# jimahlstrom/quisk

Measured on AMD Instinct MI355X. Metric: Mcomplex-samples/s through RXA chain, higher is better.
Workload: dtype f64; 1 GPU; 256 channels/GPU x 192 kHz IQ -> 48 kHz SSB RXA chain (shift + 561-tap resample/4 + adc meter + NBP nc 2048 + S meter + fixed AGC + agc meter + panel), 2^22 input samples per channel per step; meters=on, ingest=f64, channels_per_gpu=256, total_channels=256, dsp_size=256, parallelism=channel-sharded x1 (weak), no collective

## Files before the change

include/quiskhip.h:

```cpp
#ifndef QUISKHIP_H
#define QUISKHIP_H

#ifdef __cplusplus
extern "C" {
#endif

typedef enum {
    QH_OK = 0,
    QH_ERR_NO_DEVICE = -1,
    QH_ERR_INVALID = -2,
    QH_ERR_UNSUPPORTED = -3,
    QH_ERR_HIP = -4
} qh_status;

int qh_version(void);
const char *qh_last_error(void);
int qh_device_count(void);

enum { QH_LSB = 0, QH_USB, QH_DSB, QH_CWL, QH_CWU, QH_FM, QH_AM, QH_DIGU, QH_SPEC, QH_DIGL, QH_SAM, QH_DRM };

typedef struct qh_rxa qh_rxa;

qh_rxa *qh_rxa_create(int device, int nch, int dsp_size, int in_rate, int dsp_rate, int out_rate, void *stream);
void qh_rxa_destroy(qh_rxa *e);

int qh_rxa_nch(const qh_rxa *e);
int qh_rxa_dsp_insize(const qh_rxa *e);
int qh_rxa_dsp_outsize(const qh_rxa *e);
void *qh_rxa_stream(const qh_rxa *e);
int qh_rxa_set_graph_replay(qh_rxa *e, int on);
long long qh_rxa_graph_launches(const qh_rxa *e);
int qh_rxa_set_band_tile(qh_rxa *e, int nfft);
int qh_rxa_band_tile(const qh_rxa *e);

int qh_rxa_SetRXAMode(qh_rxa *e, int ch, int mode);
int qh_rxa_RXASetPassband(qh_rxa *e, int ch, double f_low, double f_high);
int qh_rxa_RXASetNC(qh_rxa *e, int ch, int nc);
int qh_rxa_SetRXAShiftRun(qh_rxa *e, int ch, int run);
int qh_rxa_SetRXAShiftFreq(qh_rxa *e, int ch, double fshift);
int qh_rxa_RXANBPSetRun(qh_rxa *e, int ch, int run);
int qh_rxa_RXANBPSetFreqs(qh_rxa *e, int ch, double flow, double fhigh);
int qh_rxa_SetRXABandpassRun(qh_rxa *e, int ch, int run);
int qh_rxa_SetRXABandpassFreqs(qh_rxa *e, int ch, double f_low, double f_high);
int qh_rxa_SetRXAAGCMode(qh_rxa *e, int ch, int mode);
int qh_rxa_SetRXAAGCFixed(qh_rxa *e, int ch, double fixed_agc_db);
int qh_rxa_SetRXAAGCAttack(qh_rxa *e, int ch, int attack_ms);
int qh_rxa_SetRXAAGCDecay(qh_rxa *e, int ch, int decay_ms);
int qh_rxa_SetRXAAGCHang(qh_rxa *e, int ch, int hang_ms);
int qh_rxa_SetRXAAGCTop(qh_rxa *e, int ch, double max_agc_db);
int qh_rxa_SetRXAAGCSlope(qh_rxa *e, int ch, int slope);
int qh_rxa_SetRXAAGCHangThreshold(qh_rxa *e, int ch, int hangthreshold);
int qh_rxa_SetRXAPanelGain1(qh_rxa *e, int ch, double gain);
int qh_rxa_SetRXAPanelGain2(qh_rxa *e, int ch, double gainI, double gainQ);
int qh_rxa_SetRXAPanelSelect(qh_rxa *e, int ch, int select);
int qh_rxa_SetRXAPanelCopy(qh_rxa *e, int ch, int copy);
int qh_rxa_SetRXAAMDSBMode(qh_rxa *e, int ch, int sbmode);
int qh_rxa_SetRXAAMDRun(qh_rxa *e, int ch, int run);
int qh_rxa_SetRXAFMLimRun(qh_rxa *e, int ch, int run);
int qh_rxa_SetRXAFMLimGain(qh_rxa *e, int ch, double gaindB);
int qh_rxa_SetEMNRTables(qh_rxa *e, const double *GG, const double *GGS, const double *zeta_hat, const int *zeta_valid, double gamma_min,
                         double gamma_max, double xi_min, double xi_max);
int qh_rxa_SetRXAEMNRRun(qh_rxa *e, int ch, int run);
int qh_rxa_SetRXAEMNRgainMethod(qh_rxa *e, int ch, int method);
int qh_rxa_SetRXAEMNRnpeMethod(qh_rxa *e, int ch, int method);
int qh_rxa_SetRXAEMNRaeRun(qh_rxa *e, int ch, int run);
int qh_rxa_SetRXAEMNRPosition(qh_rxa *e, int ch, int position);
int qh_rxa_SetRXAEMNRaeZetaThresh(qh_rxa *e, int ch, double v);
int qh_rxa_SetRXAEMNRaePsi(qh_rxa *e, int ch, double v);
int qh_rxa_SetRXAEMNRtrainZetaThresh(qh_rxa *e, int ch, double v);
int qh_rxa_SetRXAEMNRtrainT2(qh_rxa *e, int ch, double v);
int qh_rxa_SetRXAAMSQRun(qh_rxa *e, int ch, int run);
int qh_rxa_SetRXASNBARun(qh_rxa *e, int ch, int run);
int qh_rxa_SetRXASNBAOutputBandwidth(qh_rxa *e, int ch, double flow, double fhigh);
int qh_rxa_SetRXASNBAasize(qh_rxa *e, int ch, int size);
int qh_rxa_SetRXASNBAnpasses(qh_rxa *e, int ch, int npasses);
int qh_rxa_SetRXASNBAk1(qh_rxa *e, int ch, double k1);
int qh_rxa_SetRXASNBAk2(qh_rxa *e, int ch, double k2);
int qh_rxa_SetRXASNBAbridge(qh_rxa *e, int ch, int bridge);
int qh_rxa_SetRXASNBApresamps(qh_rxa *e, int ch, int presamps);
int qh_rxa_SetRXASNBApostsamps(qh_rxa *e, int ch, int postsamps);
int qh_rxa_SetRXASNBApmultmin(qh_rxa *e, int ch, double pmultmin);
int qh_rxa_SetRXASNBAovrlp(qh_rxa *e, int ch, int ovrlp);
int qh_rxa_SetRXACBLRun(qh_rxa *e, int ch, int run);
int qh_rxa_SetRXASPCWRun(qh_rxa *e, int ch, int run);
int qh_rxa_SetRXASPCWFreq(qh_rxa *e, int ch, double freq);
int qh_rxa_SetRXASPCWBandwidth(qh_rxa *e, int ch, double bw);
int qh_rxa_SetRXASPCWGain(qh_rxa *e, int ch, double gain);
int qh_rxa_SetRXAmpeakRun(qh_rxa *e, int ch, int run);
int qh_rxa_SetRXAmpeakNpeaks(qh_rxa *e, int ch, int npeaks);
int qh_rxa_SetRXAmpeakFilEnable(qh_rxa *e, int ch, int fil, int enable);
int qh_rxa_SetRXAmpeakFilFreq(qh_rxa *e, int ch, int fil, double freq);
int qh_rxa_SetRXAmpeakFilBw(qh_rxa *e, int ch, int fil, double bw);
int qh_rxa_SetRXAmpeakFilGain(qh_rxa *e, int ch, int fil, double gain);
int qh_rxa_SetRXASSQLRun(qh_rxa *e, int ch, int run);
int qh_rxa_SetRXASSQLThreshold(qh_rxa *e, int ch, double threshold);
int qh_rxa_SetRXASSQLTauMute(qh_rxa *e, int ch, double tau_mute);
int qh_rxa_SetRXASSQLTauUnMute(qh_rxa *e, int ch, double tau_unmute);
int qh_rxa_SetRXAFMSQRun(qh_rxa *e, int ch, int run);
int qh_rxa_SetRXAFMSQThreshold(qh_rxa *e, int ch, double threshold);
int qh_rxa_SetRXAFMSQNC(qh_rxa *e, int ch, int nc);
int qh_rxa_SetRXAFMSQMP(qh_rxa *e, int ch, int mp);
int qh_rxa_SetRXAEQRun(qh_rxa *e, int ch, int run);
int qh_rxa_SetRXAEQNC(qh_rxa *e, int ch, int nc);
int qh_rxa_SetRXAEQMP(qh_rxa *e, int ch, int mp);
int qh_rxa_SetRXAEQProfile(qh_rxa *e, int ch, int nfreqs, const double *F, const double *G);
int qh_rxa_SetRXAEQCtfmode(qh_rxa *e, int ch, int mode);
int qh_rxa_SetRXAEQWintype(qh_rxa *e, int ch, int wintype);
int qh_rxa_SetRXAGrphEQ(qh_rxa *e, int ch, const int *rxeq);
int qh_rxa_SetRXAGrphEQ10(qh_rxa *e, int ch, const int *rxeq);
int qh_rxa_SetRXAAMSQThreshold(qh_rxa *e, int ch, double threshold_db);
int qh_rxa_SetRXAAMSQMaxTail(qh_rxa *e, int ch, double tail_seconds);
int qh_rxa_SetRXAANFRun(qh_rxa *e, int ch, int v);
int qh_rxa_SetRXAANFTaps(qh_rxa *e, int ch, int v);
int qh_rxa_SetRXAANFDelay(qh_rxa *e, int ch, int v);
int qh_rxa_SetRXAANFPosition(qh_rxa *e, int ch, int v);
int qh_rxa_SetRXAANFGain(qh_rxa *e, int ch, double v);
// ... 681 lines not shown
```

quisk_amd/csrc/qh_engine.hip:

```cpp
#include "qh_engine.hpp"

namespace qh {

void launch_egress_pack(const double2 *src, long long src_stride, int nch, long long n, const EgressFmt &f, hipStream_t s)
{
    const long long per = (n + 255) / 256;
    hipLaunchKernelGGL(egress_pack_kernel, dim3((unsigned)(per < 1024 ? per : 1024), (unsigned)nch), dim3(256), 0, s, src, src_stride,
                       (int)n, f);
}

void Engine::pack_audio(const double2 *src, long long src_stride, long long n)
{
    launch_egress_pack(src, src_stride, nch, n, eg, stream);
}

void Engine::tick(int cat)
{
    if (!timing) return;
    if (ev_used >= (int)ev.size()) {
        hipEvent_t e;
        (void)hipEventCreate(&e);
        ev.push_back(e);
        ev_cat.push_back(0);
    }
    ev_cat[(size_t)ev_used] = cat;
    (void)hipEventRecord(ev[(size_t)ev_used], stream);
    ev_used++;
}

template <int D, bool MIX, bool PACKED = false, bool METER = false, bool OUTMIX = false, bool EGRESS = false, int NFFT = kNfft, bool POLY = false,
          int DET = 0, bool PAIR = false, bool MROW = false>
static void launch_osfir(OsfirArgs<double> a, int ntiles, int nch, hipStream_t s)
{
    a.ntiles = ntiles;
    dim3 grid((unsigned)ntiles * (unsigned)nch), block(NT);
    constexpr int lds = osfir_lds_bytes<double, NFFT, D, METER>();
    hipLaunchKernelGGL((osfir_kernel<double, NFFT, D, MIX, PACKED, METER, OUTMIX, EGRESS, POLY, DET, PAIR, MROW>), grid, block, lds, s, a);
}
template <int NFFT>
static void launch_band_rows(OsfirArgs<double> a, int ntiles, int nch, hipStream_t s)
{
    launch_osfir<1, false, false, false, false, false, NFFT, false, 0, false, true>(a, ntiles, nch, s);
}
template <int NFFT>
static void launch_band(OsfirArgs<double> a, int ntiles, int nch, hipStream_t s, bool meter, bool egress)
{
    if (meter && egress) launch_osfir<1, false, false, true, false, true, NFFT>(a, ntiles, nch, s);
    else if (meter) launch_osfir<1, false, false, true, false, false, NFFT>(a, ntiles, nch, s);
    else if (egress) launch_osfir<1, false, false, false, false, true, NFFT>(a, ntiles, nch, s);
    else launch_osfir<1, false, false, false, false, false, NFFT>(a, ntiles, nch, s);
}

static void launch_band6k(OsfirArgs<double> a, int ntiles, int nch, hipStream_t s, bool meter, bool egress)
{
    a.ntiles = ntiles;
    dim3 grid((unsigned)ntiles * (unsigned)nch), block(kOsfir6kThreads);
    constexpr int lds = osfir6k_lds_bytes();
    if (a.mask_row) hipLaunchKernelGGL((osfir6k_kernel<false, false, true>), grid, block, lds, s, a);
    else if (meter && egress) hipLaunchKernelGGL((osfir6k_kernel<true, true>), grid, block, lds, s, a);
    else if (meter) hipLaunchKernelGGL((osfir6k_kernel<true, false>), grid, block, lds, s, a);
    else if (egress) hipLaunchKernelGGL((osfir6k_kernel<false, true>), grid, block, lds, s, a);
    else hipLaunchKernelGGL((osfir6k_kernel<false, false>), grid, block, lds, s, a);
}

static void launch_band2g(OsfirArgs<double> a, int ntiles, int nch, hipStream_t s, bool meter, bool egress)
{
    a.ntiles = ntiles;
    dim3 grid((unsigned)ntiles * (unsigned)nch), block(kOsfir8kThreads);
    constexpr int lds = osfir8k_lds_bytes();
    if (a.mask_row) hipLaunchKernelGGL((osfir8k_kernel<false, false, true>), grid, block, lds, s, a);
    else if (meter && egress) hipLaunchKernelGGL((osfir8k_kernel<true, true>), grid, block, lds, s, a);
    else if (meter) hipLaunchKernelGGL((osfir8k_kernel<true, false>), grid, block, lds, s, a);
    else if (egress) hipLaunchKernelGGL((osfir8k_kernel<false, true>), grid, block, lds, s, a);
    else hipLaunchKernelGGL((osfir8k_kernel<false, false>), grid, block, lds, s, a);
}

int Engine::tile_lds_limits()
{
#define QH_SET_LDS(D, ...) QH_HIP(hipFuncSetAttribute(reinterpret_cast<const void *>(&osfir_kernel<double, 4096, D, __VA_ARGS__>), \
                                                     hipFuncAttributeMaxDynamicSharedMemorySize, (osfir_lds_bytes<double, 4096, D, true>())))
    QH_SET_LDS(1, false); QH_SET_LDS(1, false, false, true);
    QH_SET_LDS(1, false, false, false, false, true); QH_SET_LDS(1, false, false, true, false, true);
    QH_SET_LDS(1, false, false, false, false, false, false, 0, false, true); QH_SET_LDS(1, false, false, false, false, false, false, 0, true, true);
#define QH_SET_LDS8(...) QH_HIP(hipFuncSetAttribute(reinterpret_cast<const void *>(&osfir_kernel<double, kBandNfftMax, 1, false, false, __VA_ARGS__>), \
                                                     hipFuncAttributeMaxDynamicSharedMemorySize, (osfir_lds_bytes<double, kBandNfftMax, 1, true>())))
    QH_SET_LDS8(false, false, false); QH_SET_LDS8(true, false, false); QH_SET_LDS8(false, false, true); QH_SET_LDS8(true, false, true);
    QH_SET_LDS8(false, false, false, false, 0, false, true);
#undef QH_SET_LDS8
#define QH_SET_LDS6K(...) QH_HIP(hipFuncSetAttribute(reinterpret_cast<const void *>(&osfir6k_kernel<__VA_ARGS__>), \
        hipFuncAttributeMaxDynamicSharedMemorySize, osfir6k_lds_bytes()))
    QH_SET_LDS6K(false, false); QH_SET_LDS6K(true, false); QH_SET_LDS6K(false, true); QH_SET_LDS6K(true, true); QH_SET_LDS6K(false, false, true);
#undef QH_SET_LDS6K
#define QH_SET_LDS2G(...) QH_HIP(hipFuncSetAttribute(reinterpret_cast<const void *>(&osfir8k_kernel<__VA_ARGS__>), \
                                                      hipFuncAttributeMaxDynamicSharedMemorySize, osfir8k_lds_bytes()))
    QH_SET_LDS2G(false, false); QH_SET_LDS2G(true, false); QH_SET_LDS2G(false, true); QH_SET_LDS2G(true, true); QH_SET_LDS2G(false, false, true);
#undef QH_SET_LDS2G
    QH_SET_LDS(2, false, false, false, true, false, true); QH_SET_LDS(4, false, false, false, true, false, true); QH_SET_LDS(8, false, false, false, true, false, true);
    QH_SET_LDS(2, false, true, false, true, false, true); QH_SET_LDS(4, false, true, false, true, false, true); QH_SET_LDS(8, false, true, false, true, false, true);
#undef QH_SET_LDS
    if (D > 1) QH_HIP(hipFuncSetAttribute(reinterpret_cast<const void *>(&front_mask_kernel<kNfft>), hipFuncAttributeMaxDynamicSharedMemorySize,
                                          (TileFft<kNfft, false, double2>::kLdsBytes)));
    return QH_OK;
}

int Engine::emnr_lds_limit()
{
    QH_HIP(hipFuncSetAttribute(reinterpret_cast<const void *>(&emnr_kernel), hipFuncAttributeMaxDynamicSharedMemorySize, emnr_lds_bytes()));
    return QH_OK;
}

void Engine::launch_nco_retune(int n)
{
    hipLaunchKernelGGL(nco_retune_hist_kernel, dim3((kHistFront + NT - 1) / NT, (unsigned)n), dim3(NT), 0, stream,
                       hist_front[cur_front], kHistFront, nco_phase, nco_dphase, nco_parked, (const int *)retune_list,
                       (const unsigned long long *)retune_law);
}

void Engine::launch_nco_park(int ch, int run)
{
    hipLaunchKernelGGL(nco_park_kernel, dim3(1), dim3(1), 0, stream, nco_phase, nco_parked, ch, run);
}

void Engine::launch_front_masks(int n)
{
    hipLaunchKernelGGL((front_mask_kernel<kNfft>), dim3((unsigned)n), dim3(NT), (size_t)(TileFft<kNfft, false, double2>::kLdsBytes),
                       stream, (const double *)front_taps, front_ntaps, (const unsigned long long *)nco_dphase, (const int *)retune_list, front_fold,
                       (const double2 *)tw4096, mask_front, lane_rot, nco_step, 1);
}

void Engine::launch_ssql_flush()
{
    hipLaunchKernelGGL(ssql_flush_kernel, dim3((unsigned)nch), dim3(64), 0, stream, ssql_state);
}

void Engine::launch_fmsq_flush()
{
    hipLaunchKernelGGL(fmsq_flush_kernel, dim3((unsigned)((nch + 63) / 64)), dim3(64), 0, stream, fq_state, nch, fq_nready);
}

int Engine::run_front(const double2 *src, long long src_stride, double2 *dst, long long dst_stride, const EpiParam *ep,
                      long long n_in, long long n_mid, const int *list, int nlist, int part)
{
    if (part == 0) tick(0);
    if (D > 1) {
        OsfirArgs<double> a{};
        a.in = src; a.in_stride = src_stride;
        a.hist = hist_front[cur_front]; a.hist_stride = kHistFront; a.hist_len = kHistFront;
        a.out = dst; a.out_stride = dst_stride; a.out_offset = 0;
        a.mask = mask_front; a.mask_stride = kNfft;
        a.tw_fwd = tw4096; a.tw_inv = tw_inv_front;
        a.nco_step = nco_step; a.lane_rot = lane_rot;
        a.epi = ep;
        a.n_in = (int)n_in; a.n_out = (int)n_mid; a.off = 0; a.P = front_P; a.Lout = front_L; a.pick = front_pick;
        const int per_tile = front_L / front_pick;
        const int ntiles = (int)((n_mid + per_tile - 1) / per_tile);
        a.chan_list = list;
        const int nl = list ? nlist : nch;
        if (part <= 1) if (int rc = grow(tile_rot, tile_rot_cap, ntiles, nch)) return rc;
        if (part <= 1) hipLaunchKernelGGL(nco_tile_kernel, dim3((unsigned)((ntiles + 255) / 256), (unsigned)nch), dim3(256), 0, stream,
                           (const unsigned long long *)nco_phase, (const unsigned long long *)nco_dphase, tile_rot, ntiles,
                           (long long)(a.off - a.P), (long long)front_fold * front_L);
        a.tile_rot = tile_rot;
        a.pk_src = pk_src; a.pk = pk;
        const bool hist_in_kernel = !pk_src && n_in >= kHistFront && n_mid > 0;
        if (hist_in_kernel) a.hist_next = hist_front[cur_front ^ 1];
        if (part == 1 || part == 3) { }
        else if (pk_src) {
            switch (front_fold) {
            case 2: launch_osfir<2, false, true, false, true, false, kNfft, true>(a, ntiles, nl, stream); break;
            case 4: launch_osfir<4, false, true, false, true, false, kNfft, true>(a, ntiles, nl, stream); break;
            case 8: launch_osfir<8, false, true, false, true, false, kNfft, true>(a, ntiles, nl, stream); break;
            default: return set_error(QH_ERR_UNSUPPORTED, "decimation %d not supported", D);
            }
        } else {
            switch (front_fold) {
            case 2: launch_osfir<2, false, false, false, true, false, kNfft, true>(a, ntiles, nl, stream); break;
            case 4: launch_osfir<4, false, false, false, true, false, kNfft, true>(a, ntiles, nl, stream); break;
            case 8: launch_osfir<8, false, false, false, true, false, kNfft, true>(a, ntiles, nl, stream); break;
            default: return set_error(QH_ERR_UNSUPPORTED, "decimation %d not supported", D);
            }
        }
        if (part == 0) tick(2);
        if (part == 1 || part == 2) return QH_OK;
        dim3 g((kHistFront + NT - 1) / NT, (unsigned)nch);
        if (pk_src)
            hipLaunchKernelGGL((hist_update_kernel<double, false, true>), g, dim3(NT), 0, stream, src, src_stride, (int)n_in,
                               hist_front[cur_front], hist_front[cur_front ^ 1], kHistFront, (const unsigned long long *)nullptr,
                               (const unsigned long long *)nullptr, (const int *)nullptr, pk_src, pk);
        else if (!hist_in_kernel)
            hipLaunchKernelGGL((hist_update_kernel<double, false>), g, dim3(NT), 0, stream, src, src_stride, (int)n_in,
                               hist_front[cur_front], hist_front[cur_front ^ 1], kHistFront, (const unsigned long long *)nullptr,
                               (const unsigned long long *)nullptr, (const int *)nullptr, (const unsigned char *)nullptr, PackedFmt{});
        cur_front ^= 1;
    } else if (D == 0) {
        if (pk_src) return set_error(QH_ERR_UNSUPPORTED, "packed input needs in_rate / dsp_rate in 2, 4, 8, 16");
        if (int rc = grow(fbuf, fbuf_cap, n_in, nch)) return rc;
        long long per = (n_in + NT - 1) / NT;
        dim3 g((unsigned)(per < 4096 ? per : 4096), (unsigned)nch);
        hipLaunchKernelGGL((pointwise_kernel<double, true>), g, dim3(NT), 0, stream, src, src_stride, fbuf, fbuf_cap,
                           (int)n_in, nco_phase, nco_dphase, (const EpiParam *)nullptr, (const int *)nullptr);
        int got = 0;
        if (int rc = qh_rat_process(rsmpin, fbuf, fbuf_cap, (int)n_in, dst, dst_stride, &got)) return rc;
        if (got != (int)n_mid) return set_error(QH_ERR_HIP, "input resampler produced %d samples, expected %lld", got, n_mid);
        if (ep) {
            long long pm = (n_mid + NT - 1) / NT;
            hipLaunchKernelGGL((pointwise_kernel<double, false>), dim3((unsigned)(pm < 1024 ? pm : 1024), (unsigned)nch), dim3(NT), 0, stream,
                               (const double2 *)dst, dst_stride, dst, dst_stride, (int)n_mid, (const unsigned long long *)nullptr,
                               (const unsigned long long *)nullptr, ep, (const int *)nullptr);
        }
        tick(2);
    } else {
        if (pk_src) return set_error(QH_ERR_UNSUPPORTED, "packed input needs in_rate > dsp_rate (unpack with qh_unpack_iq first)");
        long long per = (n_in + NT - 1) / NT;
        dim3 g((unsigned)(per < 4096 ? per : 4096), (unsigned)nch);
        hipLaunchKernelGGL((pointwise_kernel<double, true>), g, dim3(NT), 0, stream, src, src_stride, dst, dst_stride,
                           (int)n_in, nco_phase, nco_dphase, ep, (const int *)nullptr);
        tick(2);
    }
    hipLaunchKernelGGL(nco_advance_kernel, dim3((nch + 255) / 256), dim3(256), 0, stream, nco_phase, nco_dphase, nch, n_in);
    return QH_OK;
}

static __global__ __launch_bounds__(NT) void long_gather_kernel(const double2 *hist, const double2 *src, long long src_stride, int n, double2 *cat,
                                                                long long cat_stride, const int *chan_list, int lh)
{
    const int ch = chan_list ? chan_list[blockIdx.y] : (int)blockIdx.y;
    const double2 *h = hist + (long long)ch * kLongHist, *x = src + (long long)ch * src_stride;
    double2 *c = cat + (long long)ch * cat_stride;
    const long long tot = (long long)kLongHist + n;
    for (long long i = (long long)(kLongHist - lh) + (long long)blockIdx.x * NT + threadIdx.x; i < tot; i += (long long)gridDim.x * NT) c[i] = i < kLongHist ? h[i] : x[i - kLongHist];
}
static __global__ __launch_bounds__(NT) void long_hist_kernel(const double2 *cat, long long cat_stride, int n, double2 *hist, const int *chan_list, int lh)
{
    const int ch = chan_list ? chan_list[blockIdx.y] : (int)blockIdx.y;
    const double2 *c = cat + (long long)ch * cat_stride + n;
    double2 *h = hist + (long long)ch * kLongHist;
    for (int i = kLongHist - lh + blockIdx.x * NT + threadIdx.x; i < kLongHist; i += gridDim.x * NT) h[i] = c[i];
}
static __global__ __launch_bounds__(NT) void long_add_kernel(double2 *dst, long long dst_stride, const double2 *add, long long add_stride, int n, const int *chan_list,
                                                             const int *row_parts, int row_stride, const int *mask_row, int p)
{
    const int ch = chan_list ? chan_list[blockIdx.y] : (int)blockIdx.y;
    if (p >= row_parts[mask_row ? (long long)mask_row[ch] : (long long)ch * row_stride]) return;
    double2 *d = dst + (long long)ch * dst_stride;
    const double2 *a = add + (long long)ch * add_stride;
    for (int i = blockIdx.x * NT + threadIdx.x; i < n; i += gridDim.x * NT) { d[i].x += a[i].x; d[i].y += a[i].y; }
}

static __global__ __launch_bounds__(NT) void long_migrate_kernel(double2 *hist, double2 *lhist, int to_long)
{
    const int ch = blockIdx.y;
    double2 *h = hist + (long long)ch * kHistBand, *l = lhist + (long long)ch * kLongHist;
    for (int i = blockIdx.x * NT + threadIdx.x; i < kLongHist; i += gridDim.x * NT) {
        const int j = i - (kLongHist - kHistBand);
        if (to_long) l[i] = j >= 0 ? h[j] : make_double2(0.0, 0.0);
        else if (j >= 0) h[j] = l[i];
    }
}

void Engine::run_band(const double2 *src, long long src_stride, double2 *dst, long long dst_stride, const EpiParam *ep,
// ... 7 lines not shown
        const int K = f.parts, Pk = kLongPart - 1, Lk = kBandNfftMax - Pk, nt = (int)((n_mid + Lk - 1) / Lk);
        const int nl = list ? nlist : nch;
        const long long cat_stride = kLongHist + lcat_cap;
        const int lh = K * kLongPart - 1;
        const long long per = (lh + n_mid + NT - 1) / NT;
        tick(1);
        hipLaunchKernelGGL(long_gather_kernel, dim3((unsigned)(per < 2048 ? per : 2048), (unsigned)nl), dim3(NT), 0, stream, (const double2 *)f.lhist[hc], src,
                           src_stride, (int)n_mid, lcat, cat_stride, list, lh);
        for (int p = 0; p < K; p++) {
            OsfirArgs<double> a{};
            a.in = lcat + kLongHist - (long long)kLongPart * p; a.in_stride = cat_stride;
            a.hist = a.in - Pk; a.hist_stride = cat_stride; a.hist_len = Pk;
            a.out = p ? ltmp : dst; a.out_stride = p ? lcat_cap : dst_stride; a.out_offset = 0;
            a.mask = f.lmask + (size_t)p * kBandNfftMax; a.mask_stride = f.mask_stride ? (long long)kLongParts * kBandNfftMax : 0;
            a.mask_row = f.mask_row;
            a.tw_fwd = a.tw_inv = tw8192;
            a.tw_r2 = tw8192 + 32;
            a.chan_list = list;
            a.n_in = (int)n_mid; a.n_out = (int)n_mid; a.off = 0; a.P = Pk; a.Lout = Lk;
            if (f.mask_row) launch_band_rows<kBandNfftMax>(a, nt, nl, stream);
            else launch_band<kBandNfftMax>(a, nt, nl, stream, false, false);
            const long long pn = (n_mid + NT - 1) / NT;
            if (p) hipLaunchKernelGGL(long_add_kernel, dim3((unsigned)(pn < 1024 ? pn : 1024), (unsigned)nl), dim3(NT), 0, stream, dst, dst_stride,
                                      (const double2 *)ltmp, lcat_cap, (int)n_mid, list, (const int *)f.lrow_parts, f.mask_stride ? 1 : 0, (const int *)f.mask_row, p);
        }
        const long long pn = (n_mid + NT - 1) / NT;
        if (ep) hipLaunchKernelGGL((pointwise_kernel<double, false>), dim3((unsigned)(pn < 1024 ? pn : 1024), (unsigned)nl), dim3(NT), 0, stream,
                                   (const double2 *)dst, dst_stride, dst, dst_stride, (int)n_mid, (const unsigned long long *)nullptr,
                                   (const unsigned long long *)nullptr, ep, list);
        tick(2);
        hipLaunchKernelGGL(long_hist_kernel, dim3(64, (unsigned)nl), dim3(NT), 0, stream, (const double2 *)lcat, cat_stride, (int)n_mid, f.lhist[hc ^ 1], list, lh);
        return;
    }
    const int Lout = bnfft - P;
    const int ntiles = (int)((n_mid + Lout - 1) / Lout);
    OsfirArgs<double> a{};
    a.in = src; a.in_stride = src_stride;
    a.hist = hist[hc]; a.hist_stride = kHistBand; a.hist_len = kHistBand;
    a.out = dst; a.out_stride = dst_stride; a.out_offset = 0;
    a.mask = f.mask; a.mask_stride = f.mask_stride;
    a.mask_row = f.mask_row;
    a.tw_fwd = a.tw_inv = (bnfft == kNfft || band2g) ? tw4096 : tw8192;
    a.tw_r2 = tw8192 + 32;
    a.epi = ep;
    a.chan_list = list;
    a.n_in = (int)n_mid; a.n_out = (int)n_mid; a.off = 0; a.P = P; a.Lout = Lout;
    tick(1);
    if (meter) { a.meter_in = m_part[0]; a.meter_out = m_part[1]; a.meter_stride = m_part_cap; a.meter_w = m_w; }
    if (egress) a.eg = eg;
    const int nl = list ? nlist : nch;
    const bool hist_in_kernel = !pairs && (det || (!band6k && !band2g)) && n_mid >= kHistBand;
    if (hist_in_kernel) a.hist_next = hist[hc ^ 1];
    if (pairs) {
        a.chan_list = pairs;
        if (band_fmdc) {
            a.fmdc_a = band_fmdc->a; a.fmdc_stride = band_fmdc->stride; a.fmdc_shift = band_fmdc->shift;
            a.fmdc_cin = fm_cin; a.fmdc_cstride = fm_cin_cap; a.fmdc_pw = fm_pw; a.fmdc_gain = fm_again;
        }
        if (band_amlv) {
            a.amlv_a = band_amlv->a; a.amlv_stride = band_amlv->stride; a.amlv_shift = band_amlv->shift;
            a.amlv_cin = am_cin; a.amlv_cstride = am_cin_cap; a.amlv_pw = am_pw;
        }
        if (a.mask_row) launch_osfir<1, false, false, false, false, false, kNfft, false, 0, true, true>(a, ntiles, npairs, stream);
        else launch_osfir<1, false, false, false, false, false, kNfft, false, 0, true>(a, ntiles, npairs, stream);
    } else if (det) {
        a.det_out = det_out; a.det_stride = det_stride;
        if (det == 2 || det == 3) {
            a.det_sum = am_tsum; a.det_sum_stride = am_tsum_cap;
            a.det_m[0] = am_prm.mtauR; a.det_m[1] = am_prm.mtauI;
            a.det_m256[0] = std::pow(am_prm.mtauR, 256.0); a.det_m256[1] = std::pow(am_prm.mtauI, 256.0);
            a.det_g[0] = am_prm.onem_mtauR; a.det_g[1] = am_prm.onem_mtauI;
            a.det_lf = levelfade; a.det_last = am_last; a.det_scan = am_pw + 2 * 2048;
            for (int f = 0; f < 2; f++) {
                const double m = a.det_m[f];
                a.det_mp[f][0] = m; a.det_mp[f][1] = m * m; a.det_mp[f][2] = (m * m) * (m * m); a.det_mp[f][3] = ((m * m) * (m * m)) * ((m * m) * (m * m));
            }
            if (det == 3) launch_osfir<1, false, false, false, false, false, kNfft, false, 3>(a, ntiles, nl, stream);
            else launch_osfir<1, false, false, false, false, false, kNfft, false, 2>(a, ntiles, nl, stream);
        } else launch_osfir<1, false, false, false, false, false, kNfft, false, 1>(a, ntiles, nl, stream);
    } else if (band6k) launch_band6k(a, ntiles, nl, stream, meter, egress);
    else if (band2g) launch_band2g(a, ntiles, nl, stream, meter, egress);
    else if (a.mask_row && bnfft == kNfft) launch_band_rows<kNfft>(a, ntiles, nl, stream);
    else if (a.mask_row) launch_band_rows<kBandNfftMax>(a, ntiles, nl, stream);
    else if (bnfft == kNfft) launch_band<kNfft>(a, ntiles, nl, stream, meter, egress);
    else launch_band<kBandNfftMax>(a, ntiles, nl, stream, meter, egress);
    tick(2);
    dim3 g((kHistBand + NT - 1) / NT, (unsigned)(list ? nlist : nch));
    if (pairs && band_amlv)
        hipLaunchKernelGGL(am_audio_hist_kernel, g, dim3(256), 0, stream, band_amlv->a, band_amlv->stride, (int)n_mid, list, (const double *)am_cin, am_cin_cap,
                           (const double *)am_pw, band_amlv->shift, (const double2 *)hist[hc], hist[hc ^ 1], kHistBand);
    else if (pairs && band_fmdc)
        hipLaunchKernelGGL(fm_audio_hist_kernel, g, dim3(256), 0, stream, band_fmdc->a, band_fmdc->stride, (int)n_mid, list, (const double *)fm_cin, fm_cin_cap,
                           (const double *)fm_pw, band_fmdc->shift, (const double *)fm_again, (const double2 *)hist[hc], hist[hc ^ 1], kHistBand);
    else if (!hist_in_kernel)
        hipLaunchKernelGGL((hist_update_kernel<double, false>), g, dim3(NT), 0, stream, src, src_stride, (int)n_mid,
                           hist[hc], hist[hc ^ 1], kHistBand, (const unsigned long long *)nullptr,
                           (const unsigned long long *)nullptr, list);
}

int Engine::process(const double *d_in, long long in_stride, double *d_out, long long out_stride, int nblk)
{
    if (!rsmpout) return process_chain(d_in, in_stride, d_out, out_stride, nblk);
    if (nblk <= 0) return QH_OK;
    QH_HIP(hipSetDevice(device));
    if (eg.kind) {
        const long long n_out = (long long)nblk * dsp_outsize;
        if (int rc = ensure_abuf(n_out)) return rc;
        const EgressFmt keep = eg;
        eg = EgressFmt{};
        const int rc = process(d_in, in_stride, reinterpret_cast<double *>(abuf), abuf_cap, nblk);
        eg = keep;
        if (rc) return rc;
        pack_audio(abuf, abuf_cap, n_out);
        QH_HIP(hipGetLastError());
        return QH_OK;
    }
    const long long n_mid = (long long)nblk * dsp_size;
    if (int rc = grow(obuf, obuf_cap, n_mid, nch)) return rc;
    if (int rc = process_chain(d_in, in_stride, reinterpret_cast<double *>(obuf), obuf_cap, nblk)) return rc;
    int got = 0;
    if (int rc = qh_rat_process(rsmpout, obuf, obuf_cap, (int)n_mid, d_out, out_stride, &got)) return rc;
    if (got != nblk * dsp_outsize) return set_error(QH_ERR_HIP, "output resampler produced %d samples, expected %d", got, nblk * dsp_outsize);
    return QH_OK;
}

static bool extents_apart(const double2 *a, long long a_stride, long long a_n, const double2 *b, long long b_stride, long long b_n, int nch)
{
    const double2 *a_end = a + (size_t)(nch - 1) * (size_t)a_stride + (size_t)a_n, *b_end = b + (size_t)(nch - 1) * (size_t)b_stride + (size_t)b_n;
    return (const char *)a_end <= (const char *)b || (const char *)b_end <= (const char *)a;
}

int Engine::chain_needs(ChainCall &k)
{
    for (const ChanCfg &c : cfg) {
        if (c.agc_run && c.agc_mode > 4)
            return set_error(QH_ERR_UNSUPPORTED, "AGC mode %d is not provided (0 fixed, 1-4 long/slow/med/fast)", c.agc_mode);
        if (c.amd_run && c.fmd_run) return set_error(QH_ERR_UNSUPPORTED, "channel %d: the AM and the FM detector both switched on", (int)(&c - cfg.data()));
        if (c.amd_run || c.fmd_run || (c.agc_run && c.agc_mode != 0) || c.lms[0].run || c.lms[1].run || c.amsq_run || c.emnr_run || c.snba_run || c.ap_on() || c.ssql_on()) k.mixed = true;
        if (c.sender_run || c.sip_run) k.mixed = k.taps = true;
        if (c.gen_run) {
            if (c.gen_mode == 4 || c.gen_mode == 5)
                return set_error(QH_ERR_UNSUPPORTED, "channel %d: gen0 mode %d (%s) is not provided", (int)(&c - cfg.data()), c.gen_mode, c.gen_mode == 4 ? "sawtooth" : "triangle");
            k.mixed = k.gen = true;
        }
        if (c.ssql_on() && ((int)(0.070 * dsp_rate) < 64))
            return set_error(QH_ERR_UNSUPPORTED, "SSQL needs ramps of 64 samples or more: dsp_rate %d is too low", dsp_rate);
        if (c.emnr_run && !emnr_tables) return set_error(QH_ERR_INVALID, "EMNR needs its gain tables first (qh_rxa_SetEMNRTables: WDSP's `calculus` and `zetaHat.bin` data)");
        if (c.nbp_run) { k.any_nbp = true; if (c.nbp_nc > k.nc_max) k.nc_max = c.nbp_nc; } else k.every_nbp = false;
        if (c.bp1_run) { k.any_bp1 = true; if (c.bp1_nc > k.nc_max) k.nc_max = c.bp1_nc; }
        if (c.fmd_run) {
            k.nc_max = std::max({ k.nc_max, c.fm_nc_de, c.fm_nc_aud });
            if (1.1 * c.fm_f_high >= 0.5 * (double)dsp_rate)
                return set_error(QH_ERR_UNSUPPORTED, "channel %d: FM audio band up to %g Hz needs 1.1 * high below dsp_rate / 2 = %g", (int)(&c - cfg.data()),
                                 c.fm_f_high, 0.5 * (double)dsp_rate);
        }
        if (c.fmsq_run) {
            const int ch = (int)(&c - cfg.data());
            if (!c.fmd_run) return set_error(QH_ERR_UNSUPPORTED, "channel %d: FMSQ runs while the FM detector is off", ch);
            if ((double)dsp_rate <= 2.0 * fm_pllpole(1.0, 20000.0))
                return set_error(QH_ERR_UNSUPPORTED, "FMSQ needs a dsp rate above twice the FM loop's pole frequency (%.0f Hz): %d is too low",
                                 2.0 * fm_pllpole(1.0, 20000.0), dsp_rate);
            if (c.fmsq_nc > kLongPart) return set_error(QH_ERR_UNSUPPORTED, "channel %d: FMSQ nc = %d exceeds %d", ch, c.fmsq_nc, kLongPart);
            if (c.fmsq_nc > k.nc_max) k.nc_max = c.fmsq_nc;
        }
    }
    for (const ChanCfg &c : cfg) {
        if (!c.eqp_run) continue;
// ... 47 lines not shown
        if (f.dirty) for (ChanCfg &c : cfg) c.*f.dirty = true;
        else fm_dirty = fm_relayout = true;
    }
    return QH_OK;
}

void Engine::pick_band_tile(int nc_max)
{
    const bool two_group = nc_max <= 2048 && band_tile_pref == 8192;
    const bool six_k = nc_max <= 2048 && band_tile_pref == 6144;
    const int want = six_k ? kOsfir6kN : (nc_max > 2048 || two_group) ? kBandNfftMax : kNfft;
    if (want != bnfft || two_group != band2g || six_k != band6k) {
        bnfft = want; band2g = two_group; band6k = six_k;
        for (ChanCfg &c : cfg) { c.nbp_dirty = c.bp1_dirty = true; c.snb_dirty = true; }
    }
}

int Engine::process_chain(const double *d_in, long long in_stride, double *d_out, long long out_stride, int nblk)
{
    if (nblk <= 0) return QH_OK;
    QH_HIP(hipSetDevice(device));
    ChainCall k;
    k.nblk = nblk;
    if (int rc = chain_needs(k)) return rc;
    if (int rc = plan_long(k)) return rc;
    pick_band_tile(k.nc_max);
    k.meters_fused = meters_on && !k.mixed && k.any_nbp && !k.any_bp1 && !k.any_eqp && dsp_size >= 64 && dsp_size <= 2048 && !k.long_mode;
    if (meters_on && !k.meters_fused) k.mixed = true;
    if (meters_on) if (int rc = meters_alloc()) return rc;
    if (int rc = refresh_params()) return rc;
    if (k.mixed) if (int rc = refresh_demod()) return rc;
    if (k.gen) if (int rc = refresh_gen()) return rc;
    if (!k.mixed && k.any_bp1) {
        std::vector<int> run;
        for (int ch = 0; ch < nch; ch++) if (cfg[(size_t)ch].bp1_run) run.push_back(ch);
        if (int rc = fc_follow(fc[FC_BP1], run)) return rc;
    }
    if (lists[L_SNBA].n) if (int rc = refresh_params()) return rc;
    if (k.any_eqp || eq_lists_dirty) if (int rc = refresh_eqp()) return rc;

    k.n_in = (long long)nblk * dsp_insize;
    k.n_mid = (long long)nblk * dsp_size;
    if (k.n_in > 0x7fffffffLL) return set_error(QH_ERR_INVALID, "too many samples in one call");
    if (int rc = ensure_buffers(k.n_mid)) return rc;
    if (k.long_mode) if (int rc = long_buffers()) return rc;
    if (int rc = refresh_ap(k)) return rc;
    if (int rc = refresh_ssql(k)) return rc;
    if (fq_list.n) if (int rc = grow(fq_noise, fq_noise_cap, buf_cap, nch)) return rc;
    if (k.taps && tap_lists[0].n) if (int rc = grow(snd_rows, snd_cap, buf_cap, nch)) return rc;
    snd_n = k.taps && tap_lists[0].n ? k.n_mid : 0;
    ev_used = 0;

    k.in = reinterpret_cast<const double2 *>(d_in); k.in_stride = in_stride;
    k.out = reinterpret_cast<double2 *>(d_out); k.out_stride = out_stride;
    k.P = band6k ? kOsfir6kP : band2g ? kOsfir8kP : k.meters_fused ? ((k.nc_max - 1 + 255) / 256) * 256 : k.long_mode ? kLongPart - 1 : k.nc_max - 1;
    k.eg_fused = eg.kind && (k.mixed ? lists[L_AMSQ].n == 0 : ((k.any_nbp || k.any_bp1 || k.any_eqp) && !k.long_mode));
    if (eg.kind && !k.eg_fused) {
        if (int rc = ensure_abuf(k.n_mid)) return rc;
        k.out = abuf; k.out_stride = abuf_cap;
    }
    if (!k.mixed) return run_linear(k);

    if (int rc = plan_mixed(k)) return rc;
    if (int rc = run_mixed_front(k)) return rc;
    if (int rc = run_am(k)) return rc;
    if (k.side) QH_HIP(hipEventRecord(ev_join, side_stream));
    if (lists[L_FM].n) if (int rc = run_fm(k)) return rc;
    if (k.side) QH_HIP(hipStreamWaitEvent(stream, ev_join, 0));
    if (lists[L_SNB + 1].n) snb_inplace(k, lists[L_SNB + 1].dev, lists[L_SNB + 1].n);
    if (lists[L_SNB].n || lists[L_SNB + 1].n) fc[FC_SNB].flip();
    if (int rc = run_snba(k)) return rc;
    eqp_inplace(k);
    lms_at(k, 0, k.cur);
    bp1_at(k, 0);
    tick(1);
    if (lists[L_AGC_CUR].n || lists[L_AGC_OTHER].n) if (int rc = run_agc(k)) return rc;
    run_output(k);
    QH_HIP(hipGetLastError());
    return QH_OK;
}

int Engine::run_linear(ChainCall &k)
{
    const long long n_mid = k.n_mid;
    const int nstage = 1 + (k.any_nbp ? 1 : 0) + (k.any_eqp ? 1 : 0) + (k.any_bp1 ? 1 : 0);
    int stage = 0, which = 0;
    const double2 *cur = k.in;
    long long cur_stride = k.in_stride;
    auto dst_of = [&](int st, long long &stride) -> double2 * {
        if (st == nstage - 1) { stride = k.out_stride; return k.out; }
        stride = buf_cap;
        double2 *p = buf[which];
        which ^= 1;
        return p;
    };
    {
        long long dst_stride;
        double2 *dst = dst_of(stage, dst_stride);
        const bool over = nstage == 1 && !extents_apart(k.out, k.out_stride, n_mid, k.in, k.in_stride, k.n_in, nch);
        if (over) { dst = buf[0]; dst_stride = buf_cap; }
        if (int rc = run_front(cur, cur_stride, dst, dst_stride, stage == nstage - 1 ? epi : nullptr, k.n_in, n_mid)) return rc;
        if (over) QH_HIP(hipMemcpy2DAsync(k.out, (size_t)k.out_stride * sizeof(double2), dst, (size_t)dst_stride * sizeof(double2),
                                          (size_t)n_mid * sizeof(double2), (size_t)nch, hipMemcpyDeviceToDevice, stream));
        cur = dst; cur_stride = dst_stride; stage++;
    }
    for (int f = 0; f < 3; f++) {
        if (f == 0 ? !k.any_nbp : f == 1 ? !k.any_eqp : !k.any_bp1) continue;
        long long dst_stride;
        double2 *dst = dst_of(stage, dst_stride);
        if (f == 1) {
            const bool last = stage == nstage - 1;
            run_band(cur, cur_stride, dst, dst_stride, last ? epi : nullptr, n_mid, fc[FC_EQP], k.P, eq_list.dev, eq_list.n, false, k.eg_fused && last);
            fc[FC_EQP].flip();
            if (eq_rest.n) {
                const long long per = (n_mid + NT - 1) / NT;
                const dim3 g((unsigned)(per < 1024 ? per : 1024), (unsigned)eq_rest.n);
                if (!last) hipLaunchKernelGGL(copy_rows_kernel, g, dim3(NT), 0, stream, cur, dst, buf_cap, (int)n_mid, (const int *)eq_rest.dev);
                else {
                    auto *pass = k.eg_fused ? &pointwise_kernel<double, false, true> : &pointwise_kernel<double, false>;
                    hipLaunchKernelGGL(pass, g, dim3(NT), 0, stream, cur, cur_stride, dst, dst_stride, (int)n_mid, (const unsigned long long *)nullptr,
                                       (const unsigned long long *)nullptr, (const EpiParam *)epi, (const int *)eq_rest.dev, k.eg_fused ? eg : EgressFmt{});
                }
            }
            cur = dst; cur_stride = dst_stride; stage++;
            continue;
        }
        if (k.meters_fused) if (int rc = ensure_meter_partials(n_mid, bnfft - k.P)) return rc;
        Fircore &band = fc[f == 0 ? FC_NBP : FC_BP1];
        run_band(cur, cur_stride, dst, dst_stride, stage == nstage - 1 ? epi : nullptr, n_mid, band, k.P, nullptr, 0, k.meters_fused, k.eg_fused && stage == nstage - 1);
        band.flip();
        cur = dst; cur_stride = dst_stride; stage++;
    }
    if (k.meters_fused)
        hipLaunchKernelGGL(meter_finish_kernel, dim3((unsigned)nch), dim3(kMeterFinishThreads), 0, stream, m_part[0], m_part[1],
                           m_part_cap, (int)(n_mid / 64), dsp_size / 64, (bnfft - k.P) / 64, band6k ? 2 : band2g ? 1 : 0, m_adc, m_s, m_agc,
                           -1.0 / ((double)dsp_rate * 0.100), -1.0 / ((double)dsp_rate * 0.100), (const double *)m_g2);
    if (eg.kind && !k.eg_fused) pack_audio(k.out, k.out_stride, n_mid);
    tick(3);
    QH_HIP(hipGetLastError());
    return QH_OK;
}

int Engine::plan_mixed(ChainCall &k)
{
    k.split = lists[L_FM].n > 0 && lists[L_REST].n > 0 && D > 1 && !meters_on && !k.taps && !k.gen && !lists[L_AMSQ].n && !lists[L_SNB].n && !timing && !(dbg_forms & 1);
    k.fm_theta_fused = k.split && k.any_nbp && !band6k && !band2g && bnfft == kNfft && !(dbg_forms & 8);
    bool no_lms = true;
    for (int f = 0; f < 2; f++) for (int p = 0; p < 3; p++) no_lms = no_lms && !lms_n(3 * f + p);
    k.direct = k.split && !(dbg_forms & 2) && !eq_list.n && k.every_nbp && !eg.kind && !lists[L_LIM].n && !lists[L_AGC_CUR].n && !lists[L_AGC_OTHER].n && !lists[L_SNBA].n && !lists[L_SNB + 1].n && no_lms &&
               !lists[L_EMNR].n && !lists[L_EMNR + 1].n && !lists[L_EMNR + 2].n && !lists[L_FIX].n && !lists[L_FIX + 1].n && !lists[L_BP1P + 1].n && lists[L_BP1P].n == lists[L_BP1].n && lists[L_RB].n == lists[L_BP1].n &&
               lists[L_USB].n + lists[L_FM].n == lists[L_PLAIN].n && !lists[L_AP].n && !lists[L_AP + 1].n && !ssql_listed() &&
               extents_apart(k.out, k.out_stride, k.n_mid, k.in, k.in_stride, k.n_in, nch);
    k.P_am = ((k.P + 63) / 64) * 64;
    k.am_fused = k.direct && !(dbg_forms & 4) && lists[L_AM].n > 0 && lists[L_RB].n == lists[L_AM].n + lists[L_SAM].n && !band6k && !band2g && bnfft == kNfft && k.P_am < bnfft;
    k.am_lv_fused = k.am_fused && k.P_am == 2048 && bnfft - k.P_am == 2048 && np_am > 0 && lists[L_BP1P].n && fc[FC_BP1].parts <= 1 && !(dbg_forms & (16 | 512));
    k.side = k.split || ((lists[L_AM].n || lists[L_SAM].n) && lists[L_FM].n && !(dbg_forms & 32));
    if (k.am_fused) {
        if (int rc = grow(am_tsum, am_tsum_cap, (k.n_mid + (bnfft - k.P_am) - 1) / (bnfft - k.P_am), 2LL * nch)) return rc;
        if (k.am_lv_fused) if (int rc = grow(am_cin, am_cin_cap, am_tsum_cap + 1, 2LL * nch)) return rc;
    }
    if (k.side) if (int rc = ensure_side_stream()) return rc;
    for (double *&q : seg_sum)
        if (!q) if (int rc = alloc(q, (long long)nch * kSegWaves * kSegMaxGroups * kSegSumW)) return rc;
    k.cur = buf[0]; k.other = buf[1];
    return QH_OK;
}
// ... 664 lines not shown
```

quisk_amd/csrc/qh_engine.hpp:

```cpp
#pragma once
#include <hip/hip_runtime.h>
#include <algorithm>
#include <cmath>
#include <cstdarg>
#include <cstdio>
#include <cstdlib>
#include <cstring>
#include <map>
#include <mutex>
#include <string>
#include <vector>
#include "../../include/quiskhip.h"
#include "qh_design.hpp"
#pragma clang diagnostic push
#pragma clang diagnostic ignored "-Wunused-function"
#include "qh_kernels.hpp"
#include "qh_demod.hpp"
#include "qh_tiled.hpp"
#include "qh_agc_tiled.hpp"
#include "qh_emnr.hpp"
#include "qh_snba.hpp"
#include "qh_audio_peak.hpp"
#include "qh_ssql.hpp"
#include "qh_fmsq.hpp"
// ... 65 lines not shown
    int bp1_pos = 0;
    bool demod_dirty = true, ctcss_flush = false;
    bool nbp_dirty = true, bp1_dirty = true, nco_dirty = true, epi_dirty = true;
    bool nbp_flush = false, bp1_flush = false;
    int cbl_run = 0, sp_run = 0, mp_run = 0, mp_npeaks = 2;
    double sp_f = 600.0, sp_bw = 100.0, sp_gain = 2.0;
    int mp_enable[kApPeaks] = { 1, 1 };
    double mp_f[kApPeaks] = { 2125.0, 2295.0 }, mp_bw[kApPeaks] = { 75.0, 75.0 }, mp_gain[kApPeaks] = { 1.0, 1.0 };
    bool ap_dirty = true, sp_flush = false, mp_flush[kApPeaks] = { false, false };
    bool ap_on() const { return cbl_run || sp_run || mp_run; }
    int ssql_run = 0;
    double ssql_wthresh = 0.08, ssql_tau_mute = 0.1, ssql_tau_unmute = 0.1;
    bool ssql_dirty = true;
    bool ssql_on() const { return ssql_run != 0; }
    int fmsq_run = 0, fmsq_nc = 2048, fmsq_mp = 0;
    double fmsq_tail_thresh = 0.750, fmsq_unmute_thresh = 0.562;
    bool fmsq_dirty = true;
    int eqp_run = 0, eqp_nc = 2048, eqp_mp = 0, eqp_ctfmode = 0, eqp_wintype = 0;
    std::vector<double> eqp_F = { 0.0, 32.0, 63.0, 125.0, 250.0, 500.0, 1000.0, 2000.0, 4000.0, 8000.0, 16000.0 }, eqp_G = std::vector<double>(11, 0.0);
    bool eqp_dirty = true, eqp_flush = false, eqp_tie = false;
    int sender_run = 0, sip_run = 0;
    int gen_run = 0, gen_mode = 2;
    double gen_tone_mag = 1.0, gen_tone_freq = 1000.0, gen_noise_mag = 1.0;
    double gen_sweep_mag = 1.0, gen_sweep_f1 = -20000.0, gen_sweep_f2 = 20000.0, gen_sweep_rate = 4000.0;
    unsigned long long gen_seed = 0;
    bool gen_seed_set = false, gen_dirty = true, gen_sweep_dirty = true, gen_tone_reset = false, gen_sweep_reset = false;
    bool fix_before() const
    {
        return agc_run && agc_mode == 0 && ((bp1_run && bp1_pos) || (lms[0].run && lms[0].position) || (lms[1].run && lms[1].position) ||
                                            (emnr_run && emnr_pos) || ap_on() || ssql_on());
    }
};

enum FcId { FC_NBP, FC_BP1, FC_DE, FC_AUD, FC_SNB, FC_FQ, FC_EQP, FC_COUNT };

struct Fircore {
    double2 *mask = nullptr;
    long long mask_stride = 0;
    bool by_design = false;
    int rows = 1;
    int *mask_row = nullptr;
    long long mask_rows(int nch) const { return by_design ? rows : mask_stride ? nch : 1; }
    double2 *hist[2] = { nullptr, nullptr };
    int cur = 0;
    bool ChanCfg::*dirty = nullptr;
    bool can_long = true;
    int parts = 1;
    double2 *lmask = nullptr, *lhist[2] = { nullptr, nullptr };
    int *lrow_parts = nullptr;
    struct Chan { bool listed = false, long_live = false; int at = 0; };
    std::vector<Chan> chan;
    bool carried = false;
    void flip() { cur ^= 1; }
};

struct Engine {
    int device = 0, nch = 0, dsp_size = 0, in_rate = 0, dsp_rate = 0, out_rate = 0;
    int D = 1, dsp_insize = 0, dsp_outsize = 0, front_fold = 1, front_pick = 1;
    unsigned long long epoch = 0;
    struct GraphKey {
        const void *in = nullptr; void *out = nullptr; long long in_stride = 0, out_stride = 0; int nblk = 0;
        unsigned long long epoch = ~0ull;
        bool operator==(const GraphKey &o) const
        { return in == o.in && out == o.out && in_stride == o.in_stride && out_stride == o.out_stride && nblk == o.nblk && epoch == o.epoch; }
    };
    struct GraphSlot { hipGraphExec_t exec = nullptr; unsigned after = 0; };
    bool graph_on = false, graph_seen = false;
    GraphKey graph_key;
    GraphSlot graph_slot[256];
    long long graph_launches = 0;
    hipStream_t stream = nullptr;
    bool own_stream = false;
    hipStream_t side_stream = nullptr;
    hipEvent_t ev_fork = nullptr, ev_join = nullptr;
    std::vector<ChanCfg> cfg;
    int front_ntaps = 0, front_P = 0, front_L = 0;
    double2 *mask_front = nullptr;
    double2 *tw4096 = nullptr, *tw_inv_front = nullptr, *tw8192 = nullptr;
    int bnfft = kNfft;
    bool band2g = false;
    bool band6k = false;
    int dbg_forms = [] { const char *e = std::getenv("QH_DBG_FORMS"); return e ? std::atoi(e) : 0; }();
    int band_tile_pref = 0;
    std::vector<cd> band_mask(const std::vector<cd> &h) const;
    unsigned long long *nco_phase = nullptr, *nco_dphase = nullptr, *nco_parked = nullptr;
    double2 *nco_step = nullptr;
    double2 *lane_rot = nullptr, *tile_rot = nullptr;
    long long tile_rot_cap = 0;
    double *front_taps = nullptr;
    int *retune_list = nullptr;
    unsigned long long *retune_law = nullptr;
    EpiParam *epi = nullptr;
    double2 *hist_front[2] = { nullptr, nullptr };
    int cur_front = 0;
    Fircore fc[FC_COUNT];
    double2 *buf[2] = { nullptr, nullptr };
    long long buf_cap = 0;
    double2 *lcat = nullptr, *ltmp = nullptr;
    long long lcat_cap = 0;
    int long_stage_alloc(Fircore &f);
    int long_buffers();
    int long_masks_upload(Fircore &f, long long row, const std::vector<cd> &h);
    std::map<void *, long long> owned;
    long long dev_bytes() const { long long b = 0; for (const auto &o : owned) b += o.second; return b; }
    bool timing = false;
    std::vector<hipEvent_t> ev;
    std::vector<int> ev_cat;
    int ev_used = 0;
    double last_ms[3] = { 0, 0, 0 };

    bool demod_alloc = false, lists_dirty = true;
    enum ListId {
        L_AM, L_SAM, L_FM, L_BP1, L_PLAIN, L_AGC_CUR, L_AGC_OTHER, L_LMS, L_BP1P = L_LMS + 6, L_FIX = L_BP1P + 2, L_AMSQ = L_FIX + 2, L_EMNR,
        L_SNB = L_EMNR + 3, L_SNBA = L_SNB + 2,
        L_REST,
        L_USB, L_RB,
        L_LIM, L_AP, L_PAIRS_FM = L_AP + 2, L_PAIRS_AM, L_PAIRS_SAM, L_COUNT
    };
    struct ChanList { int *dev = nullptr; int n = 0; };
    ChanList lists[L_COUNT];
    int *list_block = nullptr;
    int np_fm = 0, np_am = 0, np_sam = 0;
    bool de_real = false;
    bool all_nbp = false;
    int n_sam0 = 0;
    double *fix_gain = nullptr;
    ApParam *ap_prm = nullptr;
    double *ap_state = nullptr, *ap_M = nullptr, *ap_ends = nullptr;
    long long ap_ends_cap = 0;
    int ap_L = 0;
    std::vector<double> ap_M_h;
    std::vector<ApParam> ap_prm_h;
    int ap_alloc();
    ChanList ssql_lists[2];
    std::vector<int> ssql_h[2];
    int *ssql_list_block = nullptr;
    SsqlParam *ssql_prm = nullptr;
    SsqlState *ssql_state = nullptr;
    double *ssql_cup = nullptr, *ssql_cdown = nullptr, *ssql_ends = nullptr;
    unsigned long long *ssql_bits = nullptr;
    int *ssql_rec = nullptr;
    long long ssql_ends_cap = 0, ssql_wcap = 0, ssql_rec_cap = 0;
    int ssql_L = 0, ssql_ntup = 0, ssql_ntdown = 0;
    std::vector<SsqlParam> ssql_prm_h;
    int ssql_alloc();
    bool ssql_listed() const { return ssql_lists[0].n || ssql_lists[1].n; }
    ChanList fq_list, fq_pairs;
    std::vector<int> fq_h, fq_pairs_h;
    int *fq_list_block = nullptr;
    int np_fq = 0;
    FmsqParam *fq_prm = nullptr;
    FmsqState *fq_state = nullptr;
    double *fq_cup = nullptr, *fq_cdown = nullptr;
    double2 *fq_noise = nullptr;
    long long fq_noise_cap = 0;
    int fq_ntup = 0, fq_ntdown = 0, fq_nready = 0, fq_nc_built = 0, fq_mp_built = 0, fq_key_built = 0;
    int fmsq_alloc();
    int prm_fmsq(ChanCfg &c, int ch);
    int fmsq_filter();
    void launch_fmsq_flush();
    ChanList eq_list, eq_rest;
    std::vector<int> eq_h, eq_rest_h;
    std::vector<std::vector<cd>> eq_taps_h;
    int *eq_list_block = nullptr;
    int eq_key_built = 0;
    bool eq_lists_dirty = false;
// ... 270 lines not shown
```

quisk_amd/csrc/qh_engine_params.hip:

```cpp
#include "qh_engine.hpp"
#include <new>

namespace qh {

thread_local std::string g_last_error;

int set_error(int code, const char *fmt, ...)
{
    char buf[512];
    va_list ap;
    va_start(ap, fmt);
    vsnprintf(buf, sizeof(buf), fmt, ap);
    va_end(ap);
    g_last_error = buf;
    return code;
}

Engine::~Engine()
{
    (void)hipSetDevice(device);
    if (stream) (void)hipStreamSynchronize(stream);
    drop_graphs();
    if (rsmpout) qh_rat_destroy(rsmpout);
    if (rsmpin) qh_rat_destroy(rsmpin);
// ... 1645 lines not shown
    if (disp && qh_ana_buff_size(disp) != new_size)
        return set_error(QH_ERR_INVALID, "the attached display bank has buff_size %d: detach it before dsp_size becomes %d", qh_ana_buff_size(disp), new_size);
    QH_HIP(hipSetDevice(device));
    if (new_dsp != dsp_rate || new_size != dsp_size) return rebuild(new_in, new_dsp, new_out, new_size, new_D);
    if (int rc = quiesce()) return rc;
    if (new_in != in_rate) {
        in_rate = new_in; D = new_D;
        if (int rc = front_build()) return rc;
        if (int rc = tile_lds_limits()) return rc;
        QH_HIP(hipMemsetAsync(nco_phase, 0, (size_t)nch * sizeof(unsigned long long), stream));
        QH_HIP(hipMemsetAsync(nco_parked, 0, (size_t)nch * sizeof(unsigned long long), stream));
        for (ChanCfg &c : cfg) c.nco_dirty = true;
    }
    if (new_out != out_rate) {
        out_rate = new_out;
        if (int rc = out_build()) return rc;
    }
    QH_HIP(hipStreamSynchronize(stream));
    return QH_OK;
}

static ChanCfg settings_of(const ChanCfg &o, int dsp_rate)
{
    static_assert(sizeof(ChanCfg) == 904, "ChanCfg changed: see to settings_of, then update the size");
    ChanCfg c = o;
    const ChanCfg d;
    c.shift_on_device = d.shift_on_device;
    c.agc_dirty = d.agc_dirty; c.agc_abuf = d.agc_abuf; c.agc_rewindow = d.agc_rewindow; c.agc_ran = d.agc_ran; c.agc_stale = d.agc_stale;
    for (int f = 0; f < 2; f++) { c.lms[f].dirty = d.lms[f].dirty; c.lms[f].flush = d.lms[f].flush; }
    c.snba_flush = d.snba_flush; c.snba_taps_dirty = d.snba_taps_dirty; c.snba_rout_flush = d.snba_rout_flush; c.snb_dirty = d.snb_dirty; c.snb_flush = d.snb_flush;
    c.snba_f_low = d.snba_f_low; c.snba_f_high = d.snba_f_high;
    c.emnr_dirty = d.emnr_dirty; c.emnr_flush = d.emnr_flush; c.amsq_dirty = d.amsq_dirty;
    c.demod_dirty = d.demod_dirty; c.ctcss_flush = d.ctcss_flush;
    c.nbp_dirty = d.nbp_dirty; c.bp1_dirty = d.bp1_dirty; c.nco_dirty = d.nco_dirty; c.epi_dirty = d.epi_dirty; c.nbp_flush = d.nbp_flush; c.bp1_flush = d.bp1_flush;
    c.ap_dirty = d.ap_dirty; c.sp_flush = d.sp_flush;
    for (int i = 0; i < kApPeaks; i++) c.mp_flush[i] = d.mp_flush[i];
    c.ssql_dirty = d.ssql_dirty; c.fmsq_dirty = d.fmsq_dirty; c.lim_dirty = d.lim_dirty;
    c.fm_de_flush = d.fm_de_flush; c.fm_aud_flush = d.fm_aud_flush;
    c.eqp_dirty = d.eqp_dirty; c.eqp_flush = d.eqp_flush; c.eqp_tie = eqp_profile_tie(c.eqp_F, c.eqp_G, (double)dsp_rate);
    c.gen_dirty = d.gen_dirty; c.gen_sweep_dirty = d.gen_sweep_dirty; c.gen_tone_reset = d.gen_tone_reset; c.gen_sweep_reset = d.gen_sweep_reset;
    return c;
}

int Engine::rebuild(int new_in, int new_dsp, int new_out, int new_size, int new_D)
{
    if (int rc = quiesce()) return rc;
    if (disp_fed_pending) QH_HIP(hipEventSynchronize(disp_fed));
    const bool rate = new_dsp != dsp_rate, size = new_size != dsp_size;
    struct Line { double2 *hist[2] = { nullptr, nullptr }; int cur = 0; std::vector<Fircore::Chan> chan; long long bytes = 0; } line[FC_COUNT];
    if (!size)
        for (int s : { (int)FC_NBP, (int)FC_BP1, (int)FC_DE, (int)FC_AUD, (int)FC_EQP }) {
            Fircore &f = fc[s];
            if (!f.hist[0] || f.parts > 1) continue;
            Line &l = line[s];
            l.cur = f.cur; l.chan = f.chan; l.bytes = owned[f.hist[0]];
            for (Fircore::Chan &r : l.chan) r.long_live = false;
            for (int i = 0; i < 2; i++) { l.hist[i] = f.hist[i]; owned.erase(f.hist[i]); f.hist[i] = nullptr; }
        }
    AmState *am_keep = nullptr;
    PllState *pll_keep = nullptr;
    if (demod_alloc) { am_keep = am_state; pll_keep = pll_state; owned.erase(am_state); owned.erase(pll_state); am_state = nullptr; pll_state = nullptr; }
    Carry keep = std::move(carry);
    for (int f = 0; f < 2; f++)
        if (lms_state[f]) {
            keep.lms[f].resize(2 * (size_t)nch);
            QH_HIP(hipMemcpy2D(keep.lms[f].data(), 2 * sizeof(double), &lms_state[f][0].lidx, sizeof(LmsState), 2 * sizeof(double), (size_t)nch, hipMemcpyDeviceToHost));
        }
    if (snba_state) {
        keep.snba_frames.resize((size_t)nch * 2 * kSnbX);
        QH_HIP(hipMemcpy2D(keep.snba_frames.data(), 2 * kSnbX * sizeof(double), snba_state, (size_t)snba_prm.state_doubles * sizeof(double),
                           2 * kSnbX * sizeof(double), (size_t)nch, hipMemcpyDeviceToHost));
    }
    if (rate) keep.gen.clear();
    else if (gen_state) {
        keep.gen.resize((size_t)nch);
        QH_HIP(hipMemcpy(keep.gen.data(), gen_state, (size_t)nch * sizeof(GenState), hipMemcpyDeviceToHost));
        for (GenState &g : keep.gen) {
            const long long pos = g.pulse_pos, up = gen_pnoff, on = up + gen_pntrans, down = on + gen_pnon, T = down + gen_pntrans;
            if (pos >= up) g.pulse_pos = (long long)gen_pnoff - ((pos < on ? on : pos < down ? down : T) - pos);
        }
    }
    std::vector<ChanCfg> keep_cfg;
    for (const ChanCfg &c : cfg) keep_cfg.push_back(settings_of(c, new_dsp));
    static_assert(sizeof(Engine) == 9336, "Engine changed: see to Engine::rebuild's Wide and carried state, then update the size");
    struct Wide {
        int device, nch; hipStream_t stream; bool own_stream; unsigned long long epoch;
        bool graph_on; long long graph_launches; bool timing, meters_on; int band_tile_pref, snba_ovrlp; std::vector<SnbaTune> snba_tune_h;
        qh_ana *disp; int disp_ss, pll_check_only, agc_form;
        bool emnr_tables; std::vector<double> h_GG, h_GGS, h_zeta; std::vector<int> h_zeta_true; double h_zrange[4];
    } was{ device, nch, stream, own_stream, epoch, graph_on, graph_launches, timing, meters_on, band_tile_pref, snba_ovrlp, snba_tune_h,
           disp, disp_ss, pll_check_only, agc_form, emnr_tables, std::move(h_GG), std::move(h_GGS), std::move(h_zeta), std::move(h_zeta_true),
           { h_zrange[0], h_zrange[1], h_zrange[2], h_zrange[3] } };
    own_stream = false;
    this->~Engine();
    new (this) Engine();
    device = was.device; nch = was.nch; stream = was.stream; own_stream = was.own_stream; epoch = was.epoch + 1;
    in_rate = new_in; dsp_rate = new_dsp; out_rate = new_out; dsp_size = new_size; D = new_D;
    int rc = init();
    graph_on = was.graph_on; graph_launches = was.graph_launches; timing = was.timing; meters_on = was.meters_on;
    band_tile_pref = was.band_tile_pref; snba_ovrlp = was.snba_ovrlp; snba_tune_h = was.snba_tune_h; snba_tune_dirty = true;
    disp = was.disp; disp_ss = was.disp_ss; pll_check_only = was.pll_check_only; agc_form = was.agc_form;
    emnr_tables = was.emnr_tables; h_GG = std::move(was.h_GG); h_GGS = std::move(was.h_GGS); h_zeta = std::move(was.h_zeta); h_zeta_true = std::move(was.h_zeta_true);
    std::copy(was.h_zrange, was.h_zrange + 4, h_zrange);
    carry = std::move(keep);
    if (!rc) {
        cfg = keep_cfg;
        lists_dirty = true; eq_lists_dirty = true;
    }
    for (int s = 0; s < FC_COUNT; s++) {
        Line &l = line[s];
        if (!l.hist[0]) continue;
        Fircore &f = fc[s];
        for (int i = 0; i < 2; i++) { release(f.hist[i]); f.hist[i] = l.hist[i]; owned[l.hist[i]] = l.bytes; }
        f.cur = l.cur; f.chan = l.chan;
        f.carried = !f.mask;
    }
    if (am_keep) {
        if (!rc) rc = demod_init();
        if (!rc && !rate) {
            QH_HIP(hipMemcpyAsync(am_state, am_keep, (size_t)nch * sizeof(AmState), hipMemcpyDeviceToDevice, stream));
            QH_HIP(hipMemcpyAsync(pll_state, pll_keep, (size_t)nch * sizeof(PllState), hipMemcpyDeviceToDevice, stream));
            QH_HIP(hipStreamSynchronize(stream));
        } else if (!rc) {
            const size_t at = offsetof(PllState, dsI);
            QH_HIP(hipMemcpy2DAsync(reinterpret_cast<char *>(pll_state) + at, sizeof(PllState), reinterpret_cast<const char *>(pll_keep) + at, sizeof(PllState),
                                    sizeof(PllState) - at, (size_t)nch, hipMemcpyDeviceToDevice, stream));
            QH_HIP(hipStreamSynchronize(stream));
        }
        (void)hipFree(am_keep); (void)hipFree(pll_keep);
    }
    if (rc) return rc;
    QH_HIP(hipStreamSynchronize(stream));
    return QH_OK;
}

}
```

quisk_amd/csrc/qh_fft.hpp:

```cpp
#pragma once
#include <hip/hip_runtime.h>

namespace qh {

static constexpr double kThetaZeroMark = 8.0;


constexpr int NT = 256;

template <typename T> struct cplx_of;
template <> struct cplx_of<double> { using type = double2; };
template <> struct cplx_of<float>  { using type = float2; };
template <typename T> using cplx = typename cplx_of<T>::type;

template <typename T> __device__ __forceinline__ cplx<T> mk(T x, T y) { cplx<T> r; r.x = x; r.y = y; return r; }
template <typename C> __device__ __forceinline__ C cadd(C a, C b) { C r; r.x = a.x + b.x; r.y = a.y + b.y; return r; }
template <typename C> __device__ __forceinline__ C csub(C a, C b) { C r; r.x = a.x - b.x; r.y = a.y - b.y; return r; }
template <typename C> __device__ __forceinline__ C cmul(C a, C b)
{
    C r;
    r.x = a.x * b.x - a.y * b.y;
    r.y = a.x * b.y + a.y * b.x;
    return r;
}
// ... 45 lines not shown
        constexpr double s = (A <= 8) ? cos32(8 - A) : cos32(A - 8);
        C w;
        w.x = (T)c;
        w.y = INV ? (T)s : (T)(-s);
        return cmul(a, w);
    }
}

template <int R, bool INV, typename C> struct Dft {
    template <int I> static __device__ __forceinline__ void stage(C (&x)[R], C (&a)[R / 2], C (&b)[R / 2])
    {
        if constexpr (I < R / 2) {
            a[I] = cadd(x[I], x[I + R / 2]);
            b[I] = mul_wconst<R, I, INV>(csub(x[I], x[I + R / 2]));
            stage<I + 1>(x, a, b);
        }
    }
    static __device__ __forceinline__ void run(C (&x)[R])
    {
        C a[R / 2], b[R / 2];
        stage<0>(x, a, b);
        Dft<R / 2, INV, C>::run(a);
        Dft<R / 2, INV, C>::run(b);
#pragma unroll
        for (int q = 0; q < R / 2; q++) { x[2 * q] = a[q]; x[2 * q + 1] = b[q]; }
    }
};
template <bool INV, typename C> struct Dft<1, INV, C> { static __device__ __forceinline__ void run(C (&)[1]) {} };

__device__ __forceinline__ int lds_phys(int i) { return i + (i >> 4); }
template <int N> constexpr int lds_elems() { return N + N / 16; }

template <int R, typename C> __device__ __forceinline__ void apply_twiddle_powers(C (&x)[R], C w1)
{
    constexpr int H = R / 2 > 1 ? R / 2 : 1;
    C w[H + 1];
    w[1] = w1;
    x[1] = cmul(x[1], w1);
#pragma unroll
    for (int r = 2; r < R; r++) {
        int hi = 1;
        while (hi * 2 <= r) hi *= 2;
        const int lo = r - hi;
        C wr;
        if (hi < H || (hi == H && lo == 0)) {
            wr = (lo == 0) ? cmul(w[hi / 2], w[hi / 2]) : cmul(w[hi], w[lo]);
            w[r < H + 1 ? r : H] = wr;
        } else {
            wr = cmul(w[H], w[lo]);
        }
        x[r] = cmul(x[r], wr);
    }
}

template <int R, typename C> __device__ __forceinline__ void apply_twiddle_powers_lean(C (&x)[R], C w1)
{
    const C w2 = cmul(w1, w1);
    C we = w2, wo = w1;
    x[1] = cmul(x[1], wo);
#pragma unroll
    for (int r = 2; r < R; r++) {
        if (r & 1) { wo = cmul(wo, w2); x[r] = cmul(x[r], wo); }
        else { x[r] = cmul(x[r], we); if (r + 2 < R) we = cmul(we, w2); }
    }
}

template <int N, int R, int Ns, bool INV, typename C, bool LEAN = false>
__device__ __forceinline__ int stockham_butterfly(C (&x)[R], int j, C w1)
{
    int k = j & (Ns - 1);
    if constexpr (Ns > 1) { if constexpr (LEAN) apply_twiddle_powers_lean<R>(x, w1); else apply_twiddle_powers<R>(x, w1); }
    Dft<R, INV, C>::run(x);
    return (j - k) * R + k;
}

template <int Ns, bool INV, typename C>
__device__ __forceinline__ C pass_twiddle(const C *__restrict__ tw_pass, int j)
{
    C w = tw_pass[j & (Ns - 1)];
    return INV ? cconj(w) : w;
}

template <int N, int R, bool INV, typename C>
__device__ __forceinline__ void pass_regs_to_lds(C (&x)[R], C *lds)
{
    static_assert(R == N / NT, "first pass radix must equal N/NT");
    const int j = threadIdx.x;
    Dft<R, INV, C>::run(x);
    if constexpr (16 % R == 0) {
        C *p = lds + lds_phys(j * R);
#pragma unroll
        for (int r = 0; r < R; r++) p[r] = x[r];
    } else {
        static_assert(R % 16 == 0, "first pass radix: a divisor or a multiple of 16");
        C *p = lds + lds_phys(j * R);
#pragma unroll
        for (int r = 0; r < R; r++) p[r + r / 16] = x[r];
    }
}

template <int N, int R> struct PassGeom {
    static constexpr int NB = N / R;
    static constexpr int PER = (NB + NT - 1) / NT;
};

template <int N, int R, int Ns, bool INV, typename C>
__device__ __forceinline__ void pass_lds_to_lds(C *lds, const C (&w1)[PassGeom<N, R>::PER])
{
    constexpr int NB = PassGeom<N, R>::NB;
    constexpr int PER = PassGeom<N, R>::PER;
    C x[PER][R];
    int base[PER];
    static_assert(NB % 16 == 0, "pass geometry");
#pragma unroll
    for (int p = 0; p < PER; p++) {
        int j = threadIdx.x + p * NT;
        if (NB >= NT || j < NB) {
            const C *q = lds + lds_phys(j);
#pragma unroll
            for (int r = 0; r < R; r++) x[p][r] = q[r * (NB + NB / 16)];
        }
    }
#pragma unroll
    for (int p = 0; p < PER; p++) {
        int j = threadIdx.x + p * NT;
        if (NB >= NT || j < NB) base[p] = stockham_butterfly<N, R, Ns, INV>(x[p], j, w1[p]);
    }
    __syncthreads();
#pragma unroll
    for (int p = 0; p < PER; p++) {
        int j = threadIdx.x + p * NT;
        if (NB >= NT || j < NB) {
            if constexpr (Ns % 16 == 0) {
                C *q = lds + lds_phys(base[p]);
#pragma unroll
                for (int r = 0; r < R; r++) q[r * (Ns + Ns / 16)] = x[p][r];
            } else if constexpr (16 % (Ns * R) == 0) {
                C *q = lds + lds_phys(base[p]);
#pragma unroll
                for (int r = 0; r < R; r++) q[r * Ns] = x[p][r];
            } else {
#pragma unroll
                for (int r = 0; r < R; r++) lds[lds_phys(base[p] + r * Ns)] = x[p][r];
            }
        }
    }
}

template <int N, int R, bool INV, typename C>
__device__ __forceinline__ void pass_lds_to_regs(const C *lds, C (&x)[R], C w1)
{
    static_assert(R == N / NT, "last pass radix must equal N/NT");
    const int j = threadIdx.x;
    const C *q = lds + lds_phys(j);
#pragma unroll
    for (int r = 0; r < R; r++) x[r] = q[r * (NT + NT / 16)];
    stockham_butterfly<N, R, N / R, INV>(x, j, w1);
}

template <int N, bool INV, typename C> struct FftRR;

template <bool INV, typename C> struct FftRR<4096, INV, C> {
    struct Tw { C a[1], b; };
    static __device__ __forceinline__ Tw load(const C *__restrict__ tw) { return load_at(tw, threadIdx.x); }
    static __device__ __forceinline__ Tw load_at(const C *__restrict__ tw, int j)
    {
        Tw t;
        t.a[0] = pass_twiddle<16, INV>(tw, j);
        t.b = pass_twiddle<256, INV>(tw + 16, j);
        return t;
    }
    static __device__ __forceinline__ void first(C (&x)[16], C *lds) { pass_regs_to_lds<4096, 16, INV>(x, lds); }
    static __device__ __forceinline__ void rest(C *lds, C (&x)[16], const Tw &t)
    {
        __syncthreads();
        pass_lds_to_lds<4096, 16, 16, INV>(lds, t.a);
        __syncthreads();
        pass_lds_to_regs<4096, 16, INV>(lds, x, t.b);
    }
};

#ifndef QH_SPLIT_PAD
#define QH_SPLIT_PAD 2
#endif
#ifndef QH_SPLIT_SWIZZLE
#define QH_SPLIT_SWIZZLE 0
#endif
constexpr int split4096_lds_bytes(int scalar_bytes) { return (QH_SPLIT_SWIZZLE ? 4096 : 4096 + QH_SPLIT_PAD * 256) * scalar_bytes; }
template <bool INV, typename C> struct FftSplit4096 {
    using T = decltype(C{}.x);
    using Tw = typename FftRR<4096, INV, C>::Tw;
    static constexpr bool kSwizzle = QH_SPLIT_SWIZZLE != 0;
    template <int PHASE>
    static __device__ __forceinline__ void exchange_sw(C (&x)[16], T *lds, int j, int base)
    {
        const int m = j & 15;
        T *wb = PHASE == 1 ? lds + 16 * j : lds + (base - m);
        const T *rp = lds + 16 * (j >> 4) + (m ^ ((j >> 4) & 15));
#pragma unroll
        for (int r = 0; r < 16; r++) (PHASE == 1 ? wb : wb + 16 * r)[PHASE == 1 ? (r ^ m) : (m ^ r)] = x[r].x;
        __syncthreads();
#pragma unroll
        for (int r = 0; r < 16; r++) x[r].x = rp[256 * r];
        __syncthreads();
#pragma unroll
        for (int r = 0; r < 16; r++) (PHASE == 1 ? wb : wb + 16 * r)[PHASE == 1 ? (r ^ m) : (m ^ r)] = x[r].y;
        __syncthreads();
#pragma unroll
        for (int r = 0; r < 16; r++) x[r].y = rp[256 * r];
    }
    static constexpr int kPad = QH_SPLIT_PAD;
    static constexpr int kLdsBytes = split4096_lds_bytes((int)sizeof(T));
    static __device__ __forceinline__ int sphys(int i) { return i + (i >> 4) * kPad; }

    template <int WS, int RS, bool LB = false>
    static __device__ __forceinline__ void exchange(C (&x)[16], T *lds, int wbase, int rbase)
    {
        T *wp = lds + wbase;
        const T *rp = lds + rbase;
#pragma unroll
        for (int r = 0; r < 16; r++) wp[r * WS] = x[r].x;
        if (LB) lds_barrier(); else __syncthreads();
#pragma unroll
        for (int r = 0; r < 16; r++) x[r].x = rp[r * RS];
        if (LB) lds_barrier(); else __syncthreads();
#pragma unroll
        for (int r = 0; r < 16; r++) wp[r * WS] = x[r].y;
        if (LB) lds_barrier(); else __syncthreads();
#pragma unroll
        for (int r = 0; r < 16; r++) x[r].y = rp[r * RS];
    }

    static __device__ __forceinline__ void run(C (&x)[16], void *lds_raw, const Tw &t) { run_at(x, lds_raw, t, threadIdx.x); }
    template <bool LEAN = false>
    static __device__ __forceinline__ void run_at(C (&x)[16], void *lds_raw, const Tw &t, int j)
    {
        T *lds = reinterpret_cast<T *>(lds_raw);
        Dft<16, INV, C>::run(x);
        if constexpr (kSwizzle) exchange_sw<1>(x, lds, j, 0);
        else exchange<1, 256 + 16 * kPad>(x, lds, (16 + kPad) * j, sphys(j));
        const int base = stockham_butterfly<4096, 16, 16, INV, C, LEAN>(x, j, t.a[0]);
        __syncthreads();
        if constexpr (kSwizzle) exchange_sw<2>(x, lds, j, base);
        else exchange<16 + kPad, 256 + 16 * kPad>(x, lds, sphys(base), sphys(j));
        stockham_butterfly<4096, 16, 256, INV, C, LEAN>(x, j, t.b);
    }

    template <int D>
    static __device__ __forceinline__ void run_poly(C (&x)[16], void *lds_raw, const Tw &t)
    {
        static_assert(!INV && (D == 2 || D == 4 || D == 8), "forward transform of a decimating stage");
        constexpr int R3 = 16 / D;
        const int j = threadIdx.x;
        T *lds = reinterpret_cast<T *>(lds_raw);
        Dft<16, INV, C>::run(x);
        if constexpr (kSwizzle) exchange_sw<1>(x, lds, j, 0);
        else exchange<1, 256 + 16 * kPad>(x, lds, (16 + kPad) * j, sphys(j));
        const int base = stockham_butterfly<4096, 16, 16, INV>(x, j, t.a[0]);
        __syncthreads();
        if constexpr (kSwizzle) exchange_sw<2>(x, lds, j, base);
        else exchange<16 + kPad, 256 + 16 * kPad>(x, lds, sphys(base), sphys(j));
        C w[R3];
        w[1] = t.b;
#pragma unroll
        for (int s = 1; s < D; s <<= 1) w[1] = cmul(w[1], w[1]);
#pragma unroll
        for (int r = 2; r < R3; r++) w[r] = (r & 1) ? cmul(w[r - 1], w[1]) : cmul(w[r / 2], w[r / 2]);
        C y[16];
#pragma unroll
        for (int a = 0; a < D; a++) {
            C b[R3];
            b[0] = x[a];
#pragma unroll
            for (int r = 1; r < R3; r++) b[r] = cmul(x[a + D * r], w[r]);
            Dft<R3, INV, C>::run(b);
#pragma unroll
            for (int r = 0; r < R3; r++) y[r + R3 * a] = b[r];
        }
#pragma unroll
        for (int r = 0; r < 16; r++) x[r] = y[r];
    }
};

constexpr int kFft6kThreads = 384;
constexpr int kFft6kPad = 2;
constexpr int kFft6kLdsBytes = (6144 + 6144 / 16 * kFft6kPad) * 8;

template <bool INV, typename C> __device__ __forceinline__ void dft3(C &a, C &b, C &c)
{
    const double h = 0.86602540378443864676;
    const C t1 = cadd(b, c);
    C t2; t2.x = a.x - 0.5 * t1.x; t2.y = a.y - 0.5 * t1.y;
    const C d = csub(b, c);
    C t3;
    if (INV) { t3.x = -h * d.y; t3.y = h * d.x; } else { t3.x = h * d.y; t3.y = -h * d.x; }
    a = cadd(a, t1);
    b = cadd(t2, t3);
    c = csub(t2, t3);
}

template <int M, bool INV, typename C> __device__ __forceinline__ C mul_w24(C a)
{
    constexpr int m = M % 24;
    if constexpr (m == 0) return a;
    else if constexpr (m == 6) return mul_mi<INV>(a);
    else if constexpr (m == 12) { C r; r.x = -a.x; r.y = -a.y; return r; }
    else if constexpr (m == 18) return mul_mi<!INV>(a);
    else {
        constexpr double c15[7] = { 1.0, 0.96592582628906828675, 0.86602540378443864676, 0.70710678118654752440, 0.5,
                                    0.25881904510252076235, 0.0 };
        constexpr int q = m / 6, rem = m % 6;
        constexpr double cr = c15[rem], sr = c15[6 - rem];
        constexpr double co = q == 0 ? cr : q == 1 ? -sr : q == 2 ? -cr : sr;
        constexpr double si = q == 0 ? sr : q == 1 ? cr : q == 2 ? -sr : -cr;
        C w; w.x = co; w.y = INV ? si : -si;
        return cmul(a, w);
    }
}

template <bool INV, typename C> struct Dft24 {
    template <int N2> static __device__ __forceinline__ void tw(C (&y)[3][8])
    {
        if constexpr (N2 < 8) {
            y[1][N2] = mul_w24<N2, INV>(y[1][N2]);
            y[2][N2] = mul_w24<2 * N2, INV>(y[2][N2]);
            tw<N2 + 1>(y);
        }
    }
    static __device__ __forceinline__ void run(C (&x)[24])
    {
        C y[3][8];
#pragma unroll
        for (int n2 = 0; n2 < 8; n2++) {
            C a = x[n2], b = x[8 + n2], c = x[16 + n2];
            dft3<INV>(a, b, c);
            y[0][n2] = a; y[1][n2] = b; y[2][n2] = c;
// ... 25 lines not shown
template <bool INV> struct Fft6144 {
    using C = double2;
    static constexpr int kPad = kFft6kPad;
    static __device__ __forceinline__ int sphys(int i) { return i + (i >> 4) * kPad; }
    struct Tw { C mid, last; };
    static __device__ __forceinline__ Tw load(int t)
    {
        Tw w;
        double s, c;
        sincospi(-2.0 * (double)(t & 15) / 384.0, &s, &c);
        w.mid = make_double2(c, INV ? -s : s);
        sincospi(-2.0 * (double)t / 6144.0, &s, &c);
        w.last = make_double2(c, INV ? -s : s);
        return w;
    }
    static __device__ __forceinline__ void run(C (&x)[16], void *lds_raw, const Tw &tw, int t)
    {
        double *lds = reinterpret_cast<double *>(lds_raw);
        const bool mid = t < 256;
        Dft<16, INV, C>::run(x);
        C y[24];
        double *w1 = lds + (16 + kPad) * t;
        const double *r1 = lds + sphys(t);
#pragma unroll
        for (int r = 0; r < 16; r++) w1[r] = x[r].x;
        __syncthreads();
        if (mid) {
#pragma unroll
            for (int r = 0; r < 24; r++) y[r].x = r1[r * (256 + 16 * kPad)];
        }
        __syncthreads();
#pragma unroll
        for (int r = 0; r < 16; r++) w1[r] = x[r].y;
        __syncthreads();
        const int k = t & 15, u = t >> 4;
        double *w2 = lds + (384 + 24 * kPad) * u + k;
        if (mid) {
#pragma unroll
            for (int r = 0; r < 24; r++) y[r].y = r1[r * (256 + 16 * kPad)];
            apply_twiddle_powers24(y, tw.mid);
            Dft24<INV, C>::run(y);
        }
        __syncthreads();
        if (mid) {
#pragma unroll
            for (int r = 0; r < 24; r++) w2[r * (16 + kPad)] = y[r].x;
        }
        __syncthreads();
        const double *r2 = lds + sphys(t);
#pragma unroll
        for (int r = 0; r < 16; r++) x[r].x = r2[r * (384 + 24 * kPad)];
        __syncthreads();
        if (mid) {
#pragma unroll
            for (int r = 0; r < 24; r++) w2[r * (16 + kPad)] = y[r].y;
        }
        __syncthreads();
#pragma unroll
        for (int r = 0; r < 16; r++) x[r].y = r2[r * (384 + 24 * kPad)];
        apply_twiddle_powers<16>(x, tw.last);
        Dft<16, INV, C>::run(x);
    }
};

template <int N, bool INV, typename C> struct TileFft {
    static constexpr bool kSplit = N == 4096 && sizeof(C) == 16;
    static constexpr int kLdsBytes = kSplit ? split4096_lds_bytes(8) : lds_elems<N>() * (int)sizeof(C);
    using Tw = typename FftRR<N, INV, C>::Tw;
    static __device__ __forceinline__ Tw load(const C *__restrict__ tw) { return FftRR<N, INV, C>::load(tw); }
    static __device__ __forceinline__ void run(C (&x)[N / NT], void *lds, const Tw &t)
    {
        if constexpr (kSplit) {
            FftSplit4096<INV, C>::run(x, lds, t);
        } else {
            FftRR<N, INV, C>::first(x, reinterpret_cast<C *>(lds));
            FftRR<N, INV, C>::rest(reinterpret_cast<C *>(lds), x, t);
        }
    }
    template <int D> static __device__ __forceinline__ void run_poly(C (&x)[N / NT], void *lds, const Tw &t)
    {
        static_assert(kSplit, "polyphase plan: the fp64 4096-point transform");
        FftSplit4096<INV, C>::template run_poly<D>(x, lds, t);
    }
};

template <bool INV, typename C> struct FftRR<2048, INV, C> {
    struct Tw { C a[2], b[1], c; };
    static __device__ __forceinline__ Tw load(const C *__restrict__ tw)
    {
        Tw t;
        t.a[0] = pass_twiddle<8, INV>(tw, threadIdx.x);
        t.a[1] = pass_twiddle<8, INV>(tw, threadIdx.x + NT);
        t.b[0] = pass_twiddle<32, INV>(tw + 8, threadIdx.x);
        t.c = pass_twiddle<256, INV>(tw + 40, threadIdx.x);
        return t;
    }
    static __device__ __forceinline__ void first(C (&x)[8], C *lds) { pass_regs_to_lds<2048, 8, INV>(x, lds); }
    static __device__ __forceinline__ void rest(C *lds, C (&x)[8], const Tw &t)
    {
        __syncthreads();
        pass_lds_to_lds<2048, 4, 8, INV>(lds, t.a);
        __syncthreads();
        pass_lds_to_lds<2048, 8, 32, INV>(lds, t.b);
        __syncthreads();
        pass_lds_to_regs<2048, 8, INV>(lds, x, t.c);
    }
};

template <bool INV, typename C> struct FftRR<1024, INV, C> {
    struct Tw { C a[1], b[1], c[1], d; };
    static __device__ __forceinline__ Tw load(const C *__restrict__ tw)
    {
        Tw t;
        t.a[0] = pass_twiddle<4, INV>(tw, threadIdx.x);
        t.b[0] = pass_twiddle<16, INV>(tw + 4, threadIdx.x);
        t.c[0] = pass_twiddle<64, INV>(tw + 20, threadIdx.x);
        t.d = pass_twiddle<256, INV>(tw + 84, threadIdx.x);
        return t;
    }
    static __device__ __forceinline__ void first(C (&x)[4], C *lds) { pass_regs_to_lds<1024, 4, INV>(x, lds); }
    static __device__ __forceinline__ void rest(C *lds, C (&x)[4], const Tw &t)
    {
        __syncthreads();
        pass_lds_to_lds<1024, 4, 4, INV>(lds, t.a);
        __syncthreads();
        pass_lds_to_lds<1024, 4, 16, INV>(lds, t.b);
        __syncthreads();
        pass_lds_to_lds<1024, 4, 64, INV>(lds, t.c);
        __syncthreads();
        pass_lds_to_regs<1024, 4, INV>(lds, x, t.d);
    }
};

template <bool INV, typename C> struct FftRR<512, INV, C> {
    struct Tw { C a[1], b[1], c; };
    static __device__ __forceinline__ Tw load(const C *__restrict__ tw)
    {
        Tw t;
        t.a[0] = pass_twiddle<2, INV>(tw, threadIdx.x);
        t.b[0] = pass_twiddle<32, INV>(tw + 2, threadIdx.x);
        t.c = pass_twiddle<256, INV>(tw + 34, threadIdx.x);
        return t;
    }
    static __device__ __forceinline__ void first(C (&x)[2], C *lds) { pass_regs_to_lds<512, 2, INV>(x, lds); }
    static __device__ __forceinline__ void rest(C *lds, C (&x)[2], const Tw &t)
    {
        __syncthreads();
        pass_lds_to_lds<512, 16, 2, INV>(lds, t.a);
        __syncthreads();
        pass_lds_to_lds<512, 8, 32, INV>(lds, t.b);
        __syncthreads();
        pass_lds_to_regs<512, 2, INV>(lds, x, t.c);
    }
};

template <bool INV, typename C> struct FftRR<8192, INV, C> {
    struct Tw { C a[4], b; };
    static __device__ __forceinline__ Tw load(const C *__restrict__ tw)
    {
        Tw t;
#pragma unroll
        for (int p = 0; p < 4; p++) t.a[p] = pass_twiddle<32, INV>(tw, threadIdx.x + p * NT);
        t.b = pass_twiddle<256, INV>(tw + 32, threadIdx.x);
        return t;
    }
    static __device__ __forceinline__ void first(C (&x)[32], C *lds) { pass_regs_to_lds<8192, 32, INV>(x, lds); }
    static __device__ __forceinline__ void rest(C *lds, C (&x)[32], const Tw &t)
    {
        __syncthreads();
        pass_lds_to_lds<8192, 8, 32, INV>(lds, t.a);
        __syncthreads();
        pass_lds_to_regs<8192, 32, INV>(lds, x, t.b);
    }
};

}
```

quisk_amd/csrc/qh_osfir.hpp:

```cpp
#pragma once
#include "qh_fft.hpp"
#include "qh_wave.hpp"
#include "qh_ingest.hpp"
#include "qh_egress.hpp"

namespace qh {


struct EpiParam {
    double a, b, c, d;
};

template <typename T> struct OsfirArgs {
    const cplx<T> *in;
    const cplx<T> *hist;
    cplx<T> *hist_next;
    cplx<T> *out;
    const cplx<T> *mask;
    const cplx<T> *tw_fwd;
    const cplx<T> *tw_inv;
    const unsigned long long *nco_phase;
    const unsigned long long *nco_dphase;
    const double2 *nco_step;
    const EpiParam *epi;
// ... 10 lines not shown
    int pick;
    const unsigned char *pk_src;
    PackedFmt pk;
    const double2 *tile_rot;
    const double2 *lane_rot;
    EgressFmt eg;
    double2 *meter_in, *meter_out;
    long long meter_stride;
    const double *meter_w;
    const double2 *tw_r2;
    double *det_out;
    long long det_stride;
    double *det_sum;
    long long det_sum_stride;
    double det_m[2], det_m256[2], det_g[2];
    int pair_im0;
    const double *fmdc_a;
    long long fmdc_stride;
    const double *fmdc_cin;
    long long fmdc_cstride;
    const double *fmdc_pw;
    const double *fmdc_gain;
    int fmdc_shift;
    const int *det_lf;
    const double *det_scan;
    double det_mp[2][4];
    double *det_last;
    const double *amlv_a;
    long long amlv_stride;
    const double *amlv_cin;
    long long amlv_cstride;
    const double *amlv_pw;
    int amlv_shift;
    const int *mask_row;
};


__device__ __forceinline__ double fm_audio_at(const double *a_local, const double *cin, const double *pw, int shift, double gain, long long g)
{
    const long long t = g >> shift;
    const int k = (int)(g - (t << shift));
    return gain * __builtin_fma(-cin[t], pw[k], a_local[g]);
}

template <typename T> __device__ __forceinline__ void sincos_turns(unsigned long long ph, T &c, T &s);
template <> __device__ __forceinline__ void sincos_turns<double>(unsigned long long ph, double &c, double &s)
{
    double t = (double)(ph >> 11) * (1.0 / 9007199254740992.0);
    sincospi(2.0 * t, &s, &c);
}
template <> __device__ __forceinline__ void sincos_turns<float>(unsigned long long ph, float &c, float &s)
{
    double t = (double)(ph >> 11) * (1.0 / 9007199254740992.0);
    double sd, cd;
    sincospi(2.0 * t, &sd, &cd);
    c = (float)cd; s = (float)sd;
}

template <typename T, int E>
__device__ __forceinline__ unsigned load_tile(cplx<T> (&x)[E], const cplx<T> *__restrict__ in,
                                              const cplx<T> *__restrict__ hist, int hist_len, int n_in, int g0)
{
    using C = cplx<T>;
    const C *hsafe = hist ? hist : in;
    const int hlen = hist ? hist_len : 0;
    const int last = n_in - 1;
    unsigned okbits = 0;
#pragma unroll
    for (int r = 0; r < E; r++) {
        const int g = g0 + (int)threadIdx.x + r * NT;
        const int gi = g < 0 ? 0 : (g > last ? last : g);
        const int gh = g + hlen < 0 ? 0 : g + hlen;
        const C *p = g >= 0 ? in + gi : hsafe + (g < 0 ? gh : 0);
        const bool ok = g >= 0 ? g <= last : (g + hlen >= 0);
        okbits |= (ok ? 1u : 0u) << r;
        x[r] = *p;
    }
    return okbits;
}

#ifndef QH_XCD_SWIZZLE
#define QH_XCD_SWIZZLE 1
#endif
__device__ __forceinline__ void xcd_tile_map(int ntiles, int &chan_slot, int &tile)
{
    const unsigned G = gridDim.x, lin = blockIdx.x;
#if QH_XCD_SWIZZLE
    const unsigned c = lin & 7u, k = lin >> 3, q = G >> 3, rem = G & 7u;
    const unsigned gt = c * q + (c < rem ? c : rem) + k;
#else
    const unsigned gt = lin;
    (void)G;
#endif
    chan_slot = (int)(gt / (unsigned)ntiles);
    tile = (int)(gt - (unsigned)chan_slot * (unsigned)ntiles);
}

template <typename T, int NFFT, int D, bool METER = false> constexpr int osfir_lds_bytes()
{
    constexpr int a = TileFft<NFFT, false, cplx<T>>::kLdsBytes, b = TileFft<NFFT / D, true, cplx<T>>::kLdsBytes;
    constexpr int m = METER ? NT / 64 * 2 * 64 * 9 * 8 : 0;
    return (a > b ? a : b) > m ? (a > b ? a : b) : m;
}
template <typename T, int NFFT, int U> constexpr int osfir_interp_lds_bytes()
{
    constexpr int a = TileFft<NFFT / U, false, cplx<T>>::kLdsBytes, b = TileFft<NFFT, true, cplx<T>>::kLdsBytes;
    return a > b ? a : b;
}

#ifndef QH_MASK_BATCH
#define QH_MASK_BATCH 8
#endif
#ifndef QH_OSFIR_WAVES_F64_D1
#define QH_OSFIR_WAVES_F64_D1 4
#endif
#ifndef QH_OSFIR_WAVES_F64
#define QH_OSFIR_WAVES_F64 3
#endif
#ifndef QH_OSFIR_WAVES_F64_OUTMIX
#define QH_OSFIR_WAVES_F64_OUTMIX 3
#endif
template <typename T, int D, bool OUTMIX = false, int NFFT = 4096> constexpr int osfir_min_waves()
{
    if (NFFT >= 8192) return sizeof(T) == 8 ? 1 : 2;
    return sizeof(T) == 8 ? (D == 1 ? QH_OSFIR_WAVES_F64_D1 : OUTMIX ? QH_OSFIR_WAVES_F64_OUTMIX : QH_OSFIR_WAVES_F64) : 4;
}

#ifdef QH_OSFIR_PROBE
__device__ long long g_osfir_probe[16];
#define QH_OPROBE(slot) do { if (blockIdx.x == 7 * 8 && threadIdx.x == 0) g_osfir_probe[slot] = clock64(); } while (0)
#else
#define QH_OPROBE(slot) do { } while (0)
#endif


template <int CTRL> __device__ __forceinline__ double dpp_mov_d(double v)
{
    int lo = __double2loint(v), hi = __double2hiint(v);
    lo = __builtin_amdgcn_mov_dpp(lo, CTRL, 0xf, 0xf, false);
    hi = __builtin_amdgcn_mov_dpp(hi, CTRL, 0xf, 0xf, false);
    return __hiloint2double(hi, lo);
}
constexpr int kMeterLdsDoublesPerWave = 2 * 64 * 9;

__device__ __forceinline__ double max_nn(double a, double b)
{
    double r;
    asm("v_max_f64 %0, %1, %2" : "=v"(r) : "v"(a), "v"(b));
    return r;
}

template <typename C, int E>
__device__ __forceinline__ void meter_tap(const C (&x)[E], int r0, double wlane, double *lds_wave, double2 *dst, int wave, int lane, int wstride = -1)
{
    const int ws = wstride < 0 ? E - r0 : wstride;
    const int wr = (lane >> 3) * 9 + (lane & 7);
    const double *rd = lds_wave + lane * 9;
#pragma unroll
    for (int g = 0; g < E / 8; g++) {
        if (8 * (g + 1) <= r0) continue;
#pragma unroll
        for (int k = 0; k < 8; k++) {
            const C v = x[8 * g + k];
            double m2 = (double)v.x * (double)v.x;
            m2 = __builtin_fma((double)v.y, (double)v.y, m2);
            lds_wave[k * 72 + wr] = m2 * wlane;
            lds_wave[64 * 9 + k * 72 + wr] = m2;
        }
        __builtin_amdgcn_fence(__ATOMIC_RELEASE, "wavefront");
        __builtin_amdgcn_wave_barrier();
        __builtin_amdgcn_fence(__ATOMIC_ACQUIRE, "wavefront");
        double sum = rd[0], mx = rd[64 * 9];
#pragma unroll
        for (int k = 1; k < 8; k++) { sum += rd[k]; mx = max_nn(mx, rd[64 * 9 + k]); }
        sum += dpp_mov_d<0xB1>(sum); mx = max_nn(mx, dpp_mov_d<0xB1>(mx));
        sum += dpp_mov_d<0x4E>(sum); mx = max_nn(mx, dpp_mov_d<0x4E>(mx));
        sum += dpp_mov_d<0x141>(sum); mx = max_nn(mx, dpp_mov_d<0x141>(mx));
        const int r = 8 * g + (lane >> 3);
// ... 260 lines not shown
                if (w == wv) { kR = cR; kI = cI; }
                cR = __builtin_fma(cR, m64R, red[(4 * r + w) * 2]);
                cI = __builtin_fma(cI, m64I, red[(4 * r + w) * 2 + 1]);
            }
            const long long m = m0 + NT * r;
            if (m < a.n_out) {
                const double cR_here = sR.pw * kR, cI_here = sI.pw * kI;
                a.det_out[(long long)ch * a.det_stride + a.out_offset + m] = lf ? sv[r * NT + t] + (cI_here - cR_here) : sv[r * NT + t];
                if (m == (long long)a.n_out - 1) { a.det_last[2 * ch] = red[2 * 4 * NR] + cR_here; a.det_last[2 * ch + 1] = red[2 * 4 * NR + 1] + cI_here; }
            }
            __builtin_amdgcn_sched_barrier(0);
        }
        if (t == 0) {
            double *o = a.det_sum + ((long long)ch * a.det_sum_stride + tile) * 2;
            o[0] = lf ? cR : 0.0; o[1] = lf ? cI : 0.0;
        }
    } else if (a.pick <= 1) {
        double acc0 = 0.0, acc1 = 0.0;
#pragma unroll
        for (int i = 0; i < EO; i++) {
            const int rel = t + NT * i - j0;
            const long long m = (long long)tile * a.Lout + rel;
            double mag = 0.0;
            if (rel >= 0 && rel < a.Lout && m < a.n_out) {
                C v;
                v.x = (T)ep.a * z[i].x + (T)ep.b * z[i].y;
                v.y = (T)ep.c * z[i].x + (T)ep.d * z[i].y;
                if constexpr (DET == 1) {
                    double th = atan2((double)v.y, (double)v.x) * (1.0 / 6.2831853071795864);
                    if (v.x == (T)0 && v.y == (T)0) th = kThetaZeroMark;
                    a.det_out[(long long)ch * a.det_stride + a.out_offset + m] = th;
                } else if constexpr (DET == 2) {
                    mag = sqrt((double)v.x * (double)v.x + (double)v.y * (double)v.y);
                    a.det_out[(long long)ch * a.det_stride + a.out_offset + m] = mag;
                } else if constexpr (EGRESS) egress_store(a.eg, ch, a.out_offset + m, (double)v.x, (double)v.y);
                else out[m] = v;
            }
            if constexpr (DET == 2) {
                acc0 = __builtin_fma(acc0, a.det_m256[0], mag);
                acc1 = __builtin_fma(acc1, a.det_m256[1], mag);
            }
        }
        if constexpr (DET == 2) {
            static_assert(D == 1 && NT == 256 && !EGRESS && !METER, "the envelope tap rides on a plain D = 1 stage");
            const double s0 = wave_sum_d(acc0 * ipow_d(a.det_m[0], NT - 1 - t)), s1 = wave_sum_d(acc1 * ipow_d(a.det_m[1], NT - 1 - t));
            double *red = reinterpret_cast<double *>(lds);
            __syncthreads();
            if ((t & 63) == 0) { red[(t >> 6) * 2] = s0; red[(t >> 6) * 2 + 1] = s1; }
            __syncthreads();
            if (t == 0) {
                double *o = a.det_sum + ((long long)ch * a.det_sum_stride + tile) * 2;
                o[0] = a.det_g[0] * ((red[0] + red[2]) + (red[4] + red[6]));
                o[1] = a.det_g[1] * ((red[1] + red[3]) + (red[5] + red[7]));
            }
        }
    } else {
        const int lpt = a.Lout / a.pick;
#pragma unroll
        for (int i = 0; i < EO; i++) {
            const int rel = t + NT * i - j0;
            const int q = rel / a.pick;
            const long long m = (long long)tile * lpt + q;
            if (rel >= 0 && rel < a.Lout && q * a.pick == rel && m < a.n_out) {
                C v;
                v.x = (T)ep.a * z[i].x + (T)ep.b * z[i].y;
                v.y = (T)ep.c * z[i].x + (T)ep.d * z[i].y;
                if constexpr (EGRESS) egress_store(a.eg, ch, a.out_offset + m, (double)v.x, (double)v.y);
                else out[m] = v;
            }
        }
    }
    QH_OPROBE(5);
    if constexpr (!MIX && !PACKED && !PAIR) {
        if (a.hist_next && g0 + NFFT > a.n_in - a.hist_len) {
            C *hn = a.hist_next + (long long)ch * a.hist_stride;
            const int first = a.n_in - a.hist_len;
            const int tq = threadIdx.x;
#pragma unroll 1
            for (int g = max(g0, first) + tq; g < min(g0 + NFFT, a.n_in); g += NT) hn[g - first] = in[g];
        }
    }
}

__device__ __forceinline__ double2 sel2(bool c, double2 a, double2 b) { return make_double2(c ? a.x : b.x, c ? a.y : b.y); }
constexpr int kOsfir8kThreads = 512, kOsfir8kP = 2048, kOsfir8kLout = 6144;
constexpr int kOsfir8kImage = FftSplit4096<false, double2>::kLdsBytes > 4 * 2 * 64 * 9 * 8 ? FftSplit4096<false, double2>::kLdsBytes : 4 * 2 * 64 * 9 * 8;
constexpr int osfir8k_lds_bytes() { return 2 * kOsfir8kImage; }

template <bool METER, bool EGRESS, bool MROW = false>
__global__ __launch_bounds__(kOsfir8kThreads, 4) void osfir8k_kernel(OsfirArgs<double> a)
{
    using C = double2;
    using SF = FftSplit4096<false, C>;
    using SI = FftSplit4096<true, C>;
    constexpr int N = 8192, P = kOsfir8kP, L = kOsfir8kLout;
    extern __shared__ __align__(16) unsigned char smem8k[];
    const int T = threadIdx.x, j = T & 255;
    const int g = __builtin_amdgcn_readfirstlane(T >> 8);
    unsigned char *image = smem8k + (size_t)g * kOsfir8kImage;
    C *mine = reinterpret_cast<C *>(image), *theirs = reinterpret_cast<C *>(smem8k + (size_t)(g ^ 1) * kOsfir8kImage);
    int tile, slot;
    xcd_tile_map(a.ntiles, slot, tile);
    const int ch = a.chan_list ? a.chan_list[slot] : slot;
    const int mrow = MROW ? a.mask_row[ch] : ch;
    const C *in = a.in + (long long)ch * a.in_stride;
    const C *hist = a.hist ? a.hist + (long long)ch * a.hist_stride : nullptr;
    const int g0 = a.off - P + tile * L;
    const int n0 = 2048 * g + j;

    C x[16];
    if (g0 >= 0 && g0 + N <= a.n_in) {
        const C *p = in + g0 + n0;
#pragma unroll
        for (int s = 0; s < 8; s++) { x[s] = p[256 * s]; x[8 + s] = p[256 * s + 4096]; }
    } else {
#pragma unroll
        for (int r = 0; r < 16; r++) {
            const int gi = g0 + n0 + 256 * (r & 7) + (r >> 3) * 4096;
            C v = make_double2(0.0, 0.0);
            if (gi >= 0) { if (gi < a.n_in) v = in[gi]; }
            else if (hist && gi + a.hist_len >= 0) v = hist[gi + a.hist_len];
            x[r] = v;
        }
    }
    if constexpr (METER) {
        double *blk = reinterpret_cast<double *>(image) + (j >> 6) * kMeterLdsDoublesPerWave;
        double2 *dst = a.meter_in + (long long)ch * a.meter_stride + (long long)tile * (L >> 6) + (g ? 32 : 0);
        meter_tap<C, 16>(x, g ? 0 : 8, a.meter_w[j & 63], blk, dst, j >> 6, j & 63);
        __syncthreads();
    }

    {
        C w = a.tw_r2[j];
        if (g) w = make_double2(w.y, -w.x);
        const C wstep = make_double2(0.98078528040323044913, -0.19509032201612826785);
        C give[8];
#pragma unroll
        for (int s = 0; s < 8; s++) {
            const C sum = cadd(x[s], x[8 + s]);
            const C dif = cmul(make_double2(x[s].x - x[8 + s].x, x[s].y - x[8 + s].y), w);
            if (s < 7) w = cmul(w, wstep);
            x[s] = sel2(g != 0, dif, sum);
            give[s] = sel2(g != 0, sum, dif);
        }
#pragma unroll
        for (int s = 0; s < 8; s++) theirs[256 * s + j] = give[s];
        __syncthreads();
#pragma unroll
        for (int s = 0; s < 8; s++) {
            const C got = mine[256 * s + j], own = x[s];
            x[8 + s] = sel2(g != 0, own, got);
            x[s] = sel2(g != 0, got, own);
        }
        __syncthreads();
    }
    SF::run_at(x, image, FftRR<4096, false, C>::load_at(a.tw_fwd, j), j);

    const C *mask = a.mask + (long long)mrow * a.mask_stride + 4096 * g;
#pragma unroll
    for (int r = 0; r < 16; r++) {
        x[r] = cmul(x[r], mask[j + 256 * r]);
        if ((r + 1) % QH_MASK_BATCH == 0) __builtin_amdgcn_sched_barrier(0);
    }
    __syncthreads();
    SI::run_at(x, image, FftRR<4096, true, C>::load_at(a.tw_inv, j), j);

// ... 206 lines not shown
```

quisk_amd/csrc/qh_rxa_api.hip:

```cpp
#include "qh_engine.hpp"

using namespace qh;

extern "C" {

int qh_version(void) { return 100; }
const char *qh_last_error(void) { return g_last_error.c_str(); }

int qh_device_count(void)
{
    int n = 0;
    if (hipGetDeviceCount(&n) != hipSuccess) return 0;
    return n;
}

qh_rxa *qh_rxa_create(int device, int nch, int dsp_size, int in_rate, int dsp_rate, int out_rate, void *stream)
{
    int D = 0;
    if (nch <= 0) {
        set_error(QH_ERR_INVALID, "qh_rxa_create: bad arguments");
        return nullptr;
    }
    if (check_rates("qh_rxa_create", dsp_size, in_rate, dsp_rate, out_rate, &D)) return nullptr;
    if (qh_device_count() <= device || device < 0) {
// ... 667 lines not shown
    if (!h) return set_error(QH_ERR_INVALID, "null engine");
    QH_RXA_LOCK(h);
    if (!d_in || !d_out) return set_error(QH_ERR_INVALID, "null buffer");
    if (in_stride < (long long)nblk * h->e.dsp_insize || out_stride < (long long)nblk * h->e.dsp_outsize)
        return set_error(QH_ERR_INVALID, "stride shorter than nblk blocks");
    return h->e.process_fed(h->e.graph_on, d_in, in_stride, d_out, out_stride, nblk);
}

static long long egress_frame_bytes(const qh_audio_format *fmt)
{
    return (long long)fmt->num_channels * (fmt->kind == QH_AUDIO_I16 ? 2 : fmt->kind == QH_AUDIO_I24 ? 3 : 4);
}

static int make_egress(const qh_audio_format *fmt, void *d_out, long long out_stride_bytes, long long frames, EgressFmt *f)
{
    if (!fmt || !d_out) return set_error(QH_ERR_INVALID, "null audio format or buffer");
    if (fmt->kind < QH_AUDIO_I16 || fmt->kind > QH_AUDIO_F32) return set_error(QH_ERR_INVALID, "audio kind %d", fmt->kind);
    if (fmt->num_channels < 1 || fmt->channel_I < 0 || fmt->channel_Q < 0 || fmt->channel_I >= fmt->num_channels ||
        fmt->channel_Q >= fmt->num_channels)
        return set_error(QH_ERR_INVALID, "audio channel slots outside the frame");
    const int bytes = egress_frame_bytes(fmt) / fmt->num_channels;
    if (out_stride_bytes < frames * fmt->num_channels * bytes) return set_error(QH_ERR_INVALID, "audio row stride shorter than the frames");
    if (fmt->kind != QH_AUDIO_I24 && out_stride_bytes % bytes) return set_error(QH_ERR_INVALID, "audio row stride not a multiple of the sample size");
    f->kind = fmt->kind; f->nchan = fmt->num_channels; f->ch_i = fmt->channel_I; f->ch_q = fmt->channel_Q;
    f->volume = fmt->volume; f->prescale = fmt->prescale == 0.0 ? 1.0 : fmt->prescale;
    f->out = static_cast<unsigned char *>(d_out); f->stride = out_stride_bytes;
    return QH_OK;
}

int qh_rxa_process_audio(qh_rxa *h, const double *d_in, long long in_stride, void *d_out, long long out_stride_bytes, int nblk,
                         const qh_audio_format *fmt)
{
    if (!h) return set_error(QH_ERR_INVALID, "null engine");
    QH_RXA_LOCK(h);
    if (!d_in) return set_error(QH_ERR_INVALID, "null buffer");
    if (in_stride < (long long)nblk * h->e.dsp_insize) return set_error(QH_ERR_INVALID, "stride shorter than nblk blocks");
    EgressFmt f{};
    if (int rc = make_egress(fmt, d_out, out_stride_bytes, (long long)nblk * h->e.dsp_outsize, &f)) return rc;
    if (rows_overlap(d_in, in_stride * 16, (long long)nblk * h->e.dsp_insize * 16, d_out, out_stride_bytes,
                     (long long)nblk * h->e.dsp_outsize * egress_frame_bytes(fmt), h->e.nch))
        return set_error(QH_ERR_INVALID, "qh_rxa_process_audio: the output rows overlap the input rows (in place is not supported)");
    h->e.eg = f;
    const int rc = h->e.process_fed(false, d_in, in_stride, nullptr, 0, nblk);
    h->e.eg = EgressFmt{};
    return rc;
}

int qh_audio_pack(int device, void *stream, const double *d_src, long long src_stride, int nch, int n, const qh_audio_format *fmt,
                  void *d_dst, long long dst_stride_bytes)
{
    if (!d_src || nch <= 0 || n < 0) return set_error(QH_ERR_INVALID, "qh_audio_pack: bad arguments");
    if (qh_device_count() <= device || device < 0) return set_error(QH_ERR_NO_DEVICE, "no HIP device %d (libquiskhip has no CPU fallback)", device);
    EgressFmt f{};
    if (int rc = make_egress(fmt, d_dst, dst_stride_bytes, n, &f)) return rc;
    if (n == 0) return QH_OK;
    if (rows_overlap(d_src, src_stride * 16, (long long)n * 16, d_dst, dst_stride_bytes, (long long)n * egress_frame_bytes(fmt), nch))
        return set_error(QH_ERR_INVALID, "qh_audio_pack: the output rows overlap the input rows (in place is not supported)");
    QH_HIP(hipSetDevice(device));
    launch_egress_pack(reinterpret_cast<const double2 *>(d_src), src_stride, nch, n, f, (hipStream_t)stream);
    QH_HIP(hipGetLastError());
    return QH_OK;
}

int qh_rxa_set_graph_replay(qh_rxa *h, int on)
{
    if (!h) return set_error(QH_ERR_INVALID, "null engine");
    QH_RXA_LOCK(h);
    h->e.graph_on = on != 0;
    if (!on) { h->e.drop_graphs(); h->e.graph_key = Engine::GraphKey{}; }
    return QH_OK;
}
long long qh_rxa_graph_launches(const qh_rxa *h) { return h ? h->e.graph_launches : 0; }

int qh_rxa_set_band_tile(qh_rxa *h, int nfft)
{
    if (!h || (nfft != 0 && nfft != 4096 && nfft != 6144 && nfft != 8192)) return set_error(QH_ERR_INVALID, "qh_rxa_set_band_tile: 0 (default), 4096, 6144 or 8192");
    QH_RXA_LOCK(h);
    h->e.band_tile_pref = nfft;
    h->e.epoch++;
    return QH_OK;
}
int qh_rxa_band_tile(const qh_rxa *h) { return h ? h->e.bnfft : 0; }

int qh_rxa_process_packed(qh_rxa *h, const void *d_src, long long src_bytes, const qh_iq_format *fmt, long long chan_stride,
                          double *d_out, long long out_stride, int nblk)
{
    if (!h) return set_error(QH_ERR_INVALID, "null engine");
    QH_RXA_LOCK(h);
    if (!d_src || !d_out || !fmt) return set_error(QH_ERR_INVALID, "null buffer");
    if (out_stride < (long long)nblk * h->e.dsp_outsize) return set_error(QH_ERR_INVALID, "stride shorter than nblk blocks");
    PackedFmt pk;
    if (int rc = qh::make_packed_fmt(fmt, chan_stride, src_bytes, (long long)nblk * h->e.dsp_insize, h->e.nch, &pk)) return rc;
    if (rows_overlap(d_src, 0, src_bytes, d_out, out_stride * 16, (long long)nblk * h->e.dsp_outsize * 16, h->e.nch))
        return set_error(QH_ERR_INVALID, "qh_rxa_process_packed: the output rows overlap the packed source (in place is not supported)");
    h->e.pk_src = static_cast<const unsigned char *>(d_src);
    h->e.pk = pk;
    const int rc = h->e.process_fed(false, reinterpret_cast<const double *>(d_src), (long long)nblk * h->e.dsp_insize, d_out, out_stride, nblk);
    h->e.pk_src = nullptr;
    return rc;
}

int qh_rxa_flush(qh_rxa *h)
{
    if (!h) return set_error(QH_ERR_INVALID, "null engine");
    QH_RXA_LOCK(h);
    return h->e.flush();
}

int qh_rxa_set_sender(qh_rxa *h, int ch, int run)
{
    if (h && h->e.disp && !run) return set_error(QH_ERR_INVALID, "qh_rxa_set_sender: a display is attached (qh_rxa_attach_display), it reads every channel's rows");
    FOR_CH(h, ch, { run = run ? 1 : 0; if (c.sender_run != run) { c.sender_run = run; h->e.lists_dirty = true; } });
}

int qh_rxa_sender_rows(qh_rxa *h, const float **d_rows, long long *stride, int *n)
{
    if (!h || !d_rows || !stride || !n) return set_error(QH_ERR_INVALID, "qh_rxa_sender_rows: null argument");
    QH_RXA_LOCK(h);
    *d_rows = reinterpret_cast<const float *>(h->e.snd_rows); *stride = h->e.snd_cap; *n = (int)h->e.snd_n;
    return QH_OK;
}

int qh_rxa_sender_rows_host(qh_rxa *h, int ch, float *out, int max, int *n)
{
    if (!h || !out || !n) return set_error(QH_ERR_INVALID, "qh_rxa_sender_rows_host: null argument");
    QH_RXA_LOCK(h);
    Engine &e = h->e;
    if (ch < 0 || ch >= e.nch) return set_error(QH_ERR_INVALID, "channel %d out of range", ch);
    if (!e.cfg[(size_t)ch].sender_run) return set_error(QH_ERR_INVALID, "channel %d: the sender is off (qh_rxa_set_sender)", ch);
    *n = (int)e.snd_n;
    if (e.snd_n > max) return set_error(QH_ERR_INVALID, "qh_rxa_sender_rows_host: %lld samples, room for %d", e.snd_n, max);
    if (e.snd_n == 0) return QH_OK;
    QH_HIP(hipSetDevice(e.device));
    QH_HIP(hipMemcpyAsync(out, e.snd_rows + (size_t)ch * (size_t)e.snd_cap, (size_t)e.snd_n * sizeof(float2), hipMemcpyDeviceToHost, e.stream));
    QH_HIP(hipStreamSynchronize(e.stream));
    return QH_OK;
}

int qh_rxa_set_siphon(qh_rxa *h, int ch, int run)
{
    FOR_CH(h, ch, {
        run = run ? 1 : 0;
        if (c.sip_run == run) continue;
        c.sip_run = run; h->e.lists_dirty = true;
        if (run && h->e.sip_ring) {
            QH_HIP(hipSetDevice(h->e.device));
            QH_HIP(hipMemsetAsync(h->e.sip_ring + (size_t)_i * kSipSize, 0, (size_t)kSipSize * sizeof(double2), h->e.stream));
            QH_HIP(hipMemsetAsync(h->e.sip_idx + _i, 0, sizeof(int), h->e.stream));
        }
    });
}

int qh_rxa_get_sip(qh_rxa *h, int ch, double *out, int size)
{
    if (!h || !out) return set_error(QH_ERR_INVALID, "qh_rxa_get_sip: null argument");
    QH_RXA_LOCK(h);
    Engine &e = h->e;
    if (ch < 0 || ch >= e.nch) return set_error(QH_ERR_INVALID, "channel %d out of range", ch);
    if (size < 0 || size > kSipSize) return set_error(QH_ERR_INVALID, "qh_rxa_get_sip: size %d outside 0 .. %d", size, kSipSize);
    if (!e.cfg[(size_t)ch].sip_run) return set_error(QH_ERR_INVALID, "channel %d: the siphon is off (qh_rxa_set_siphon)", ch);
    if (size == 0) return QH_OK;
    if (!e.sip_ring) { std::memset(out, 0, (size_t)size * 2 * sizeof(double)); return QH_OK; }
    QH_HIP(hipSetDevice(e.device));
    QH_HIP(hipStreamSynchronize(e.stream));
    int idx = 0;
    QH_HIP(hipMemcpy(&idx, e.sip_idx + ch, sizeof(int), hipMemcpyDeviceToHost));
// ... 274 lines not shown
```

quisk_amd/lib.py:

```python
import ctypes as C
import os

_HERE = os.path.dirname(os.path.abspath(__file__))
LIB_PATH = os.environ.get("QUISKHIP_LIB") or os.path.join(_HERE, "lib", "libquiskhip.so")
_lib = None


class QuiskHipError(RuntimeError):
    pass


def load():
    global _lib
    if _lib is not None:
        return _lib
    if not os.path.exists(LIB_PATH):
        raise QuiskHipError(
            "%s is missing: build it with `python -m quisk_amd.build` (needs hipcc). "
            "quisk_amd has no CPU fallback." % LIB_PATH)
    L = C.CDLL(LIB_PATH)
    vp, i, d, ll = C.c_void_p, C.c_int, C.c_double, C.c_longlong
    L.qh_version.restype = i
    L.qh_last_error.restype = C.c_char_p
    L.qh_device_count.restype = i
# ... 1 lines not shown
    L.qh_rxa_create.argtypes = [i, i, i, i, i, i, vp]
    L.qh_rxa_destroy.argtypes = [vp]
    L.qh_rxa_destroy.restype = None
    for n in ("qh_rxa_nch", "qh_rxa_dsp_insize", "qh_rxa_dsp_outsize"):
        getattr(L, n).argtypes = [vp]
        getattr(L, n).restype = i
    L.qh_rxa_device_bytes.argtypes = [vp]
    L.qh_rxa_device_bytes.restype = ll
    for n in ("SetRXAMode", "RXASetNC", "SetRXAShiftRun", "RXANBPSetRun", "SetRXABandpassRun", "SetRXAAGCMode",
              "SetRXAPanelSelect", "SetRXAPanelCopy", "SetRXAAMDSBMode", "SetRXAAMDFadeLevel", "SetRXACTCSSRun",
              "SetRXAAGCAttack", "SetRXAAGCDecay", "SetRXAAGCHang", "SetRXAAGCSlope", "SetRXAAGCHangThreshold",
              "RXASetMP", "SetRXAAMDRun", "SetRXAFMLimRun", "RXANBPSetNotchesRun", "RXANBPSetWindow", "RXANBPSetAutoIncrease",
              "SetRXAEMNRRun", "SetRXAEMNRgainMethod", "SetRXAEMNRnpeMethod", "SetRXAEMNRaeRun", "SetRXAEMNRPosition", "SetRXASNBARun", "SetRXASNBAasize", "SetRXASNBAnpasses", "SetRXASNBAbridge", "SetRXASNBApresamps", "SetRXASNBApostsamps", "SetRXASNBAovrlp",
              "SetRXAAMSQRun", "SetRXAANFRun", "SetRXAANFTaps", "SetRXAANFDelay", "SetRXAANFPosition", "SetRXAANRRun", "SetRXAANRTaps", "SetRXAANRDelay",
              "SetRXAANRPosition"):
        f = getattr(L, "qh_rxa_" + n)
        f.argtypes = [vp, i, i]
        f.restype = i
    L.qh_rxa_RXANBPAddNotch.argtypes = [vp, i, i, d, d, i, C.POINTER(i)]
    L.qh_rxa_RXANBPEditNotch.argtypes = [vp, i, i, d, d, i, C.POINTER(i)]
    L.qh_rxa_RXANBPDeleteNotch.argtypes = [vp, i, i, C.POINTER(i)]
    L.qh_rxa_RXANBPGetNotch.argtypes = [vp, i, i, C.POINTER(d), C.POINTER(d), C.POINTER(i), C.POINTER(i)]
    L.qh_rxa_RXANBPGetNumNotches.argtypes = [vp, i, C.POINTER(i)]
    L.qh_rxa_RXANBPGetMinNotchWidth.argtypes = [vp, i, C.POINTER(d)]
    for n in ("SetRXAShiftFreq", "SetRXAAGCFixed", "SetRXAPanelGain1", "SetRXAFMDeviation", "SetRXACTCSSFreq", "SetRXAAGCTop",
              "RXANBPSetTuneFrequency", "RXANBPSetShiftFrequency", "SetRXAFMLimGain", "SetRXAAMSQThreshold", "SetRXAAMSQMaxTail", "SetRXAEMNRaeZetaThresh", "SetRXAEMNRaePsi", "SetRXAEMNRtrainZetaThresh", "SetRXASNBAk1", "SetRXASNBAk2", "SetRXASNBApmultmin",
              "SetRXAEMNRtrainT2", "SetRXAANFGain", "SetRXAANFLeakage",
              "SetRXAANRGain", "SetRXAANRLeakage"):
        f = getattr(L, "qh_rxa_" + n)
        f.argtypes = [vp, i, d]
        f.restype = i
    for n in ("RXASetPassband", "RXANBPSetFreqs", "SetRXABandpassFreqs", "SetRXAPanelGain2", "SetRXASNBAOutputBandwidth"):
        f = getattr(L, "qh_rxa_" + n)
        f.argtypes = [vp, i, d, d]
        f.restype = i
    for n in ("SetRXAANFVals", "SetRXAANRVals"):
        getattr(L, "qh_rxa_" + n).argtypes = [vp, i, i, i, d, d]
    for n, a in (("SetRXACBLRun", [vp, i, i]), ("SetRXASPCWRun", [vp, i, i]), ("SetRXASPCWFreq", [vp, i, d]),
                 ("SetRXASPCWBandwidth", [vp, i, d]), ("SetRXASPCWGain", [vp, i, d]), ("SetRXAmpeakRun", [vp, i, i]),
                 ("SetRXAmpeakNpeaks", [vp, i, i]), ("SetRXAmpeakFilEnable", [vp, i, i, i]), ("SetRXAmpeakFilFreq", [vp, i, i, d]),
                 ("SetRXAmpeakFilBw", [vp, i, i, d]), ("SetRXAmpeakFilGain", [vp, i, i, d]),
                 ("SetRXASSQLRun", [vp, i, i]), ("SetRXASSQLThreshold", [vp, i, d]), ("SetRXASSQLTauMute", [vp, i, d]),
                 ("SetRXASSQLTauUnMute", [vp, i, d]),
                 ("SetRXAFMSQRun", [vp, i, i]), ("SetRXAFMSQThreshold", [vp, i, d]), ("SetRXAFMSQNC", [vp, i, i]), ("SetRXAFMSQMP", [vp, i, i]),
                 ("SetRXAEQRun", [vp, i, i]), ("SetRXAEQNC", [vp, i, i]), ("SetRXAEQMP", [vp, i, i]),
                 ("SetRXAEQProfile", [vp, i, i, C.POINTER(d), C.POINTER(d)]), ("SetRXAEQCtfmode", [vp, i, i]), ("SetRXAEQWintype", [vp, i, i]),
                 ("SetRXAGrphEQ", [vp, i, C.POINTER(i)]), ("SetRXAGrphEQ10", [vp, i, C.POINTER(i)])):
        f = getattr(L, "qh_rxa_" + n)
        f.argtypes = a
        f.restype = i
    for n, a in (("SetRXAFMSQRun", [i, i]), ("SetRXAFMSQThreshold", [i, d]), ("SetRXAFMSQNC", [i, i]), ("SetRXAFMSQMP", [i, i])):
        f = getattr(L, n)
        f.argtypes = a
        f.restype = None
    for n, a in (("SetRXAEQRun", [i, i]), ("SetRXAEQNC", [i, i]), ("SetRXAEQMP", [i, i]), ("SetRXAEQProfile", [i, i, C.POINTER(d), C.POINTER(d)]),
                 ("SetRXAEQCtfmode", [i, i]), ("SetRXAEQWintype", [i, i]), ("SetRXAGrphEQ", [i, C.POINTER(i)]), ("SetRXAGrphEQ10", [i, C.POINTER(i)])):
        f = getattr(L, n)
        f.argtypes = a
        f.restype = None
    for n, a in (("SetRXAFMAFFilter", [i, d, d]), ("SetRXAFMNCde", [i, i]), ("SetRXAFMMPde", [i, i]), ("SetRXAFMNCaud", [i, i]), ("SetRXAFMMPaud", [i, i])):
        f = getattr(L, "qh_rxa_" + n)
        f.argtypes = [vp] + a
        f.restype = i
        f = getattr(L, n)
        f.argtypes = a
        f.restype = None
    L.qh_rxa_debug_fm_rows.argtypes = [vp, C.POINTER(i), C.POINTER(i), C.POINTER(ll)]
    L.qh_rxa_debug_fm_rows.restype = i
    L.qh_rxa_debug_eqp.argtypes = [vp, i, C.POINTER(d), i]
    L.qh_rxa_debug_eqp.restype = i
    L.qh_rxa_debug_fmsq.argtypes = [vp, i, C.POINTER(d), i]
    L.qh_rxa_debug_fmsq.restype = i
    L.qh_rxa_SetEMNRTables.argtypes = [vp, vp, vp, vp, vp, d, d, d, d]
    L.qh_rxa_process.argtypes = [vp, vp, ll, vp, ll, i]
    L.qh_rxa_process.restype = i
    L.qh_rxa_process_host.argtypes = [vp, vp, ll, vp, ll, i]
    L.qh_rxa_process_host.restype = i
    L.qh_rxa_synchronize.argtypes = [vp]
    L.qh_rxa_synchronize.restype = i
    L.qh_rxa_enable_meters.argtypes = [vp, i]
    L.qh_rxa_set_graph_replay.argtypes = [vp, i]
    L.qh_rxa_set_band_tile.argtypes = [vp, i]
    L.qh_rxa_band_tile.argtypes = [vp]
    L.qh_rxa_graph_launches.argtypes = [vp]
    L.qh_rxa_graph_launches.restype = ll
    L.qh_rxa_pll_repairs.argtypes = [vp]
    L.qh_rxa_pll_repairs.restype = ll
    L.qh_rxa_debug_agc.argtypes = [vp, i]
    L.qh_rxa_debug_agc.restype = i
    L.qh_rxa_agc_repairs.argtypes = [vp]
    L.qh_rxa_agc_repairs.restype = ll
    L.qh_rxa_agc_segments_rerun.argtypes = [vp]
    L.qh_rxa_agc_segments_rerun.restype = ll
    L.qh_rxa_agc_tiled_channels.argtypes = [vp]
    L.qh_rxa_agc_tiled_channels.restype = i
    L.qh_rxa_process_audio.argtypes = [vp, vp, ll, vp, ll, i, vp]
    L.qh_rxa_process_audio.restype = i
    L.qh_audio_pack.argtypes = [i, vp, vp, ll, i, i, vp, vp, ll]
    L.qh_audio_pack.restype = i
    L.qh_wdsp_graph_launches.restype = ll
    L.qh_wdsp_fexchange0_device.argtypes = [i, vp, i, vp]
    L.qh_wdsp_fexchange0_device.restype = i
    L.qh_rxa_GetRXAMeter.argtypes = [vp, i, i, C.POINTER(d)]
    L.qh_rxa_set_sender.argtypes = [vp, i, i]
    L.qh_rxa_sender_rows.argtypes = [vp, C.POINTER(vp), C.POINTER(ll), C.POINTER(i)]
    L.qh_rxa_sender_rows_host.argtypes = [vp, i, vp, i, C.POINTER(i)]
    L.qh_rxa_set_siphon.argtypes = [vp, i, i]
    L.qh_rxa_get_sip.argtypes = [vp, i, vp, i]
    L.qh_rxa_attach_display.argtypes = [vp, vp, i]
    L.qh_rxa_feed_display.argtypes = [vp, vp, i]
    L.SetRXASpectrum.argtypes = [i, i, i, i, i]
    L.SetRXASpectrum.restype = None
    L.RXAGetaSipF.argtypes = [i, vp, i]
    L.RXAGetaSipF.restype = None
    L.RXAGetaSipF1.argtypes = [i, vp, i]
    L.RXAGetaSipF1.restype = None
    for n in ("Run", "Mode"):
        getattr(L, "qh_rxa_SetRXAPreGen" + n).argtypes = [vp, i, i]
        getattr(L, "SetRXAPreGen" + n).argtypes = [i, i]
        getattr(L, "SetRXAPreGen" + n).restype = None
    for n in ("ToneMag", "ToneFreq", "NoiseMag", "SweepMag", "SweepRate"):
        getattr(L, "qh_rxa_SetRXAPreGen" + n).argtypes = [vp, i, d]
        getattr(L, "SetRXAPreGen" + n).argtypes = [i, d]
        getattr(L, "SetRXAPreGen" + n).restype = None
    L.qh_rxa_SetRXAPreGenSweepFreq.argtypes = [vp, i, d, d]
    L.SetRXAPreGenSweepFreq.argtypes = [i, d, d]
    L.SetRXAPreGenSweepFreq.restype = None
    L.qh_rxa_set_gen_seed.argtypes = [vp, i, C.c_ulonglong]
    L.qh_rxa_flush.argtypes = [vp]
    L.qh_rxa_flush.restype = i
    for n in ("qh_rxa_in_rate", "qh_rxa_dsp_rate", "qh_rxa_out_rate", "qh_rxa_dsp_size"):
        getattr(L, n).argtypes = [vp]
        getattr(L, n).restype = i
    L.qh_rxa_set_rates.argtypes = [vp, i, i, i]
    for n in ("qh_rxa_set_in_rate", "qh_rxa_set_dsp_rate", "qh_rxa_set_out_rate", "qh_rxa_set_dsp_size"):
        getattr(L, n).argtypes = [vp, i]
    for n in ("SetType", "SetInputBuffsize", "SetDSPBuffsize", "SetInputSamplerate", "SetDSPSamplerate", "SetOutputSamplerate"):
        getattr(L, n).argtypes = [i, i]
        getattr(L, n).restype = None
    L.SetAllRates.argtypes = [i, i, i, i]
    L.SetAllRates.restype = None
    for n in ("SetChannelTDelayUp", "SetChannelTSlewUp", "SetChannelTDelayDown", "SetChannelTSlewDown"):
        getattr(L, n).argtypes = [i, d]
        getattr(L, n).restype = None
    L.qh_rxa_enable_timing.argtypes = [vp, i]
    L.qh_rxa_enable_timing.restype = i
    L.qh_rxa_timing.argtypes = [vp, C.POINTER(d), i]
    L.qh_rxa_timing.restype = i
    L.qh_fir_create.restype = vp
    L.qh_fir_create.argtypes = [i, i, vp, vp, i, i, i, vp]
    L.qh_fir_destroy.argtypes = [vp]
    L.qh_fir_destroy.restype = None
    L.qh_fir_reset.argtypes = [vp]
    L.qh_fir_out_count.argtypes = [vp, i]
    L.qh_fir_process.argtypes = [vp, vp, ll, i, vp, ll, C.POINTER(i)]
    L.qh_fir_process_host.argtypes = [vp, vp, ll, i, vp, ll, C.POINTER(i)]
    L.qh_fir_synchronize.argtypes = [vp]
    L.qh_rat_create.restype = vp
    L.qh_rat_create.argtypes = [i, i, vp, i, i, i, i, vp]
    L.qh_rat_destroy.argtypes = [vp]
    L.qh_rat_destroy.restype = None
    L.qh_rat_reset.argtypes = [vp]
    L.qh_rat_set_state.argtypes = [vp, vp, i]
    L.qh_rat_phase.argtypes = [vp]
    L.qh_rat_out_count.argtypes = [vp, i]
    L.qh_rat_process.argtypes = [vp, vp, ll, i, vp, ll, C.POINTER(i)]
# ... 293 lines not shown
```

quisk_amd/rxa.py:

```python
import ctypes as C

import numpy as np

from .lib import load, check, QuiskHipError

_SETTERS = ("SetRXAMode", "RXASetNC", "SetRXAShiftRun", "RXANBPSetRun", "SetRXABandpassRun", "SetRXAAGCMode",
            "SetRXAPanelSelect", "SetRXAPanelCopy", "SetRXAShiftFreq", "SetRXAAGCFixed", "SetRXAPanelGain1",
            "RXASetPassband", "RXANBPSetFreqs", "SetRXABandpassFreqs", "SetRXAPanelGain2", "SetRXAAMDSBMode",
            "SetRXAAMDFadeLevel", "SetRXAFMDeviation", "SetRXACTCSSFreq", "SetRXACTCSSRun", "SetRXAAGCAttack",
            "SetRXAAGCDecay", "SetRXAAGCHang", "SetRXAAGCTop", "SetRXAAGCSlope", "SetRXAAGCHangThreshold", "RXASetMP",
            "SetRXAAMDRun", "RXANBPSetNotchesRun", "RXANBPSetWindow", "RXANBPSetAutoIncrease", "RXANBPSetTuneFrequency",
            "RXANBPSetShiftFrequency", "SetRXAFMLimRun", "SetRXAFMLimGain",
            "SetRXASNBARun", "SetRXASNBAOutputBandwidth", "SetRXASNBAasize", "SetRXASNBAnpasses", "SetRXASNBAk1", "SetRXASNBAk2", "SetRXASNBAbridge", "SetRXASNBApresamps", "SetRXASNBApostsamps", "SetRXASNBApmultmin", "SetRXASNBAovrlp", "SetRXAEMNRRun", "SetRXAEMNRgainMethod", "SetRXAEMNRnpeMethod", "SetRXAEMNRaeRun", "SetRXAEMNRPosition", "SetRXAEMNRaeZetaThresh", "SetRXAEMNRaePsi", "SetRXAEMNRtrainZetaThresh", "SetRXAEMNRtrainT2",
            "SetRXAAMSQRun", "SetRXAAMSQThreshold", "SetRXAAMSQMaxTail", "SetRXAANFRun", "SetRXAANFTaps", "SetRXAANFDelay", "SetRXAANFPosition", "SetRXAANFGain", "SetRXAANFLeakage", "SetRXAANFVals",
            "SetRXAANRRun", "SetRXAANRTaps", "SetRXAANRDelay", "SetRXAANRPosition", "SetRXAANRGain", "SetRXAANRLeakage", "SetRXAANRVals",
            "SetRXACBLRun", "SetRXASPCWRun", "SetRXASPCWFreq", "SetRXASPCWBandwidth", "SetRXASPCWGain", "SetRXAmpeakRun",
            "SetRXAmpeakNpeaks", "SetRXAmpeakFilEnable", "SetRXAmpeakFilFreq", "SetRXAmpeakFilBw", "SetRXAmpeakFilGain",
            "SetRXASSQLRun", "SetRXASSQLThreshold", "SetRXASSQLTauMute", "SetRXASSQLTauUnMute",
            "SetRXAFMSQRun", "SetRXAFMSQThreshold", "SetRXAFMSQNC", "SetRXAFMSQMP",
            "SetRXAFMAFFilter", "SetRXAFMNCde", "SetRXAFMMPde", "SetRXAFMNCaud", "SetRXAFMMPaud",
            "SetRXAEQRun", "SetRXAEQNC", "SetRXAEQMP", "SetRXAEQProfile", "SetRXAEQCtfmode", "SetRXAEQWintype", "SetRXAGrphEQ", "SetRXAGrphEQ10")
_ARRAYS = {"SetRXAEQProfile": ((C.c_double, 1), (C.c_double, 2)), "SetRXAGrphEQ": ((C.c_int, 0),), "SetRXAGrphEQ10": ((C.c_int, 0),)}


# ... 130 lines not shown
    def get_sip(self, ch, size):
        out = np.zeros(max(int(size), 0), dtype=np.complex128)
        check(self._L.qh_rxa_get_sip(self._h, ch, out.ctypes.data if out.size else np.zeros(1, dtype=np.complex128).ctypes.data, int(size)))
        return out

    def attach_display(self, bank, ss=0):
        check(self._L.qh_rxa_attach_display(self._h, bank._h if bank is not None else None, ss))
        self._display = bank

    def SetRXAPreGenRun(self, ch, run):
        check(self._L.qh_rxa_SetRXAPreGenRun(self._h, ch, 1 if run else 0))

    def SetRXAPreGenMode(self, ch, mode):
        check(self._L.qh_rxa_SetRXAPreGenMode(self._h, ch, int(mode)))

    def SetRXAPreGenToneMag(self, ch, mag):
        check(self._L.qh_rxa_SetRXAPreGenToneMag(self._h, ch, float(mag)))

    def SetRXAPreGenToneFreq(self, ch, freq):
        check(self._L.qh_rxa_SetRXAPreGenToneFreq(self._h, ch, float(freq)))

    def SetRXAPreGenNoiseMag(self, ch, mag):
        check(self._L.qh_rxa_SetRXAPreGenNoiseMag(self._h, ch, float(mag)))

    def SetRXAPreGenSweepMag(self, ch, mag):
        check(self._L.qh_rxa_SetRXAPreGenSweepMag(self._h, ch, float(mag)))

    def SetRXAPreGenSweepFreq(self, ch, freq1, freq2):
        check(self._L.qh_rxa_SetRXAPreGenSweepFreq(self._h, ch, float(freq1), float(freq2)))

    def SetRXAPreGenSweepRate(self, ch, rate):
        check(self._L.qh_rxa_SetRXAPreGenSweepRate(self._h, ch, float(rate)))

    def set_gen_seed(self, ch, seed):
        check(self._L.qh_rxa_set_gen_seed(self._h, ch, int(seed) & 0xFFFFFFFFFFFFFFFF))

    def pll_repairs(self):
        return self._L.qh_rxa_pll_repairs(self._h)

    def debug_fmsq(self, ch):
        buf = (C.c_double * 5)()
        n = self._L.qh_rxa_debug_fmsq(self._h, ch, buf, 5)
        check(n if n < 0 else 0)
        return (buf[0], buf[1], int(buf[2]), int(buf[3]), int(buf[4])) if n == 5 else None

    def debug_fm_rows(self):
        de, au, n = C.c_int(0), C.c_int(0), C.c_longlong(0)
        check(self._L.qh_rxa_debug_fm_rows(self._h, C.byref(de), C.byref(au), C.byref(n)))
        return de.value, au.value, n.value

    def debug_eqp(self, ch, max_nc=4096):
        buf = (C.c_double * (2 * max_nc))()
        n = self._L.qh_rxa_debug_eqp(self._h, ch, buf, 2 * max_nc)
        check(n if n < 0 else 0)
        return np.frombuffer(buf, dtype=np.complex128, count=n).copy() if n > 0 else None

    def debug_agc(self, form):
        check(self._L.qh_rxa_debug_agc(self._h, int(form)))

    def agc_repairs(self):
        return self._L.qh_rxa_agc_repairs(self._h)

    def agc_segments_rerun(self):
        return self._L.qh_rxa_agc_segments_rerun(self._h)

    def agc_tiled_channels(self):
        return self._L.qh_rxa_agc_tiled_channels(self._h)

    def synchronize(self):
        check(self._L.qh_rxa_synchronize(self._h))

    def flush(self):
        check(self._L.qh_rxa_flush(self._h))

    def set_graph_replay(self, on=True):
        check(self._L.qh_rxa_set_graph_replay(self._h, 1 if on else 0))

    def set_band_tile(self, nfft=0):
        check(self._L.qh_rxa_set_band_tile(self._h, int(nfft)))

    def band_tile(self):
        return self._L.qh_rxa_band_tile(self._h)

    def graph_launches(self):
        return self._L.qh_rxa_graph_launches(self._h)

    def enable_timing(self, on=True):
        check(self._L.qh_rxa_enable_timing(self._h, 1 if on else 0))

    def timing_ms(self):
        buf = (C.c_double * 3)()
        n = self._L.qh_rxa_timing(self._h, buf, 3)
        return [buf[k] for k in range(n)]

    def device_bytes(self):
        return self._L.qh_rxa_device_bytes(self._h)

    def _resized(self, rc):
        check(rc)
        self.dsp_insize = self._L.qh_rxa_dsp_insize(self._h)
        self.dsp_outsize = self._L.qh_rxa_dsp_outsize(self._h)

    def set_rates(self, in_rate, dsp_rate, out_rate):
        self._resized(self._L.qh_rxa_set_rates(self._h, int(in_rate), int(dsp_rate), int(out_rate)))

    def set_in_rate(self, in_rate):
        self._resized(self._L.qh_rxa_set_in_rate(self._h, int(in_rate)))

    def set_dsp_rate(self, dsp_rate):
        self._resized(self._L.qh_rxa_set_dsp_rate(self._h, int(dsp_rate)))

    def set_out_rate(self, out_rate):
        self._resized(self._L.qh_rxa_set_out_rate(self._h, int(out_rate)))

    def set_dsp_size(self, dsp_size):
        self._resized(self._L.qh_rxa_set_dsp_size(self._h, int(dsp_size)))

    @property
    def in_rate(self):
        return self._L.qh_rxa_in_rate(self._h)

    @property
    def dsp_rate(self):
        return self._L.qh_rxa_dsp_rate(self._h)

    @property
    def out_rate(self):
        return self._L.qh_rxa_out_rate(self._h)

    @property
    def dsp_size(self):
        return self._L.qh_rxa_dsp_size(self._h)

    def close(self):
        if getattr(self, "_h", None):
            self._L.qh_rxa_destroy(self._h)
            self._h = None

    def __del__(self):
        try:
            self.close()
        except Exception:
            pass
```

Measured before the change: 146,600 Mcomplex-samples/s.

## Add persistent tile-walk kernel for decimating front FIR stage

Adds a persistent-workgroup variant of the overlap-save FIR kernel. It launches only as many workgroups as can be resident, sized from an occupancy query, and has each one loop over tiles. Twiddle factors are loaded once and carried across iterations in registers. It is enabled by default for the D=4 polyphase front stage, while the band stage variant is compiled but disabled by macro. The goal is to cut per-workgroup launch and twiddle reload overhead, at the cost of higher register pressure and possible load imbalance across the tail of the tile walk.

```diff
diff --git a/include/quiskhip.h b/include/quiskhip.h
--- a/include/quiskhip.h
+++ b/include/quiskhip.h
@@ -32,6 +32,7 @@
 long long qh_rxa_graph_launches(const qh_rxa *e);
 int qh_rxa_set_band_tile(qh_rxa *e, int nfft);
 int qh_rxa_band_tile(const qh_rxa *e);
+int qh_rxa_set_tile_walk(qh_rxa *e, int on, int max_workgroups);
 
 int qh_rxa_SetRXAMode(qh_rxa *e, int ch, int mode);
 int qh_rxa_RXASetPassband(qh_rxa *e, int ch, double f_low, double f_high);
diff --git a/quisk_amd/csrc/qh_engine.hip b/quisk_amd/csrc/qh_engine.hip
--- a/quisk_amd/csrc/qh_engine.hip
+++ b/quisk_amd/csrc/qh_engine.hip
@@ -36,6 +36,16 @@
     dim3 grid((unsigned)ntiles * (unsigned)nch), block(NT);
     constexpr int lds = osfir_lds_bytes<double, NFFT, D, METER>();
     hipLaunchKernelGGL((osfir_kernel<double, NFFT, D, MIX, PACKED, METER, OUTMIX, EGRESS, POLY, DET, PAIR, MROW>), grid, block, lds, s, a);
+}
+template <int D, bool METER, bool OUTMIX, bool POLY>
+static void launch_walk(OsfirArgs<double> a, int ntiles, int nch, int resident, hipStream_t s)
+{
+    a.ntiles = ntiles;
+    const int total = ntiles * nch;
+    int g = resident >= 8 ? resident & ~7 : resident;
+    if (g > total) g = total;
+    constexpr int lds = osfir_lds_bytes<double, kNfft, D, METER>();
+    hipLaunchKernelGGL((osfir_walk_kernel<double, kNfft, D, METER, OUTMIX, POLY>), dim3((unsigned)g), dim3(NT), lds, s, a, total);
 }
 template <int NFFT>
 static void launch_band_rows(OsfirArgs<double> a, int ntiles, int nch, hipStream_t s)
@@ -100,6 +110,19 @@
 #undef QH_SET_LDS
     if (D > 1) QH_HIP(hipFuncSetAttribute(reinterpret_cast<const void *>(&front_mask_kernel<kNfft>), hipFuncAttributeMaxDynamicSharedMemorySize,
                                           (TileFft<kNfft, false, double2>::kLdsBytes)));
+    int cus = 0;
+    QH_HIP(hipDeviceGetAttribute(&cus, hipDeviceAttributeMultiprocessorCount, device));
+    const void *walk[3] = { reinterpret_cast<const void *>(&osfir_walk_kernel<double, kNfft, 4, false, true, true>),
+                            reinterpret_cast<const void *>(&osfir_walk_kernel<double, kNfft, 1, false, false, false>),
+                            reinterpret_cast<const void *>(&osfir_walk_kernel<double, kNfft, 1, true, false, false>) };
+    const int walk_lds[3] = { osfir_lds_bytes<double, kNfft, 4, false>(), osfir_lds_bytes<double, kNfft, 1, false>(), osfir_lds_bytes<double, kNfft, 1, true>() };
+    for (int i = 0; i < 3; i++) {
+        int per_cu = 0;
+        QH_HIP(hipFuncSetAttribute(walk[i], hipFuncAttributeMaxDynamicSharedMemorySize, walk_lds[i]));
+        QH_HIP(hipOccupancyMaxActiveBlocksPerMultiprocessor(&per_cu, walk[i], NT, (size_t)walk_lds[i]));
+        walk_res[i] = per_cu * cus;
+        if (walk_res[i] <= 0) return set_error(QH_ERR_HIP, "tile walk: no resident workgroup (occupancy query)");
+    }
     return QH_OK;
 }
 
@@ -175,7 +198,10 @@
         } else {
             switch (front_fold) {
             case 2: launch_osfir<2, false, false, false, true, false, kNfft, true>(a, ntiles, nl, stream); break;
-            case 4: launch_osfir<4, false, false, false, true, false, kNfft, true>(a, ntiles, nl, stream); break;
+            case 4:
+                if (walk_now && QH_TILE_WALK_FRONT && part == 0) launch_walk<4, false, true, true>(a, ntiles, nl, walk_grid(0), stream);
+                else launch_osfir<4, false, false, false, true, false, kNfft, true>(a, ntiles, nl, stream);
+                break;
             case 8: launch_osfir<8, false, false, false, true, false, kNfft, true>(a, ntiles, nl, stream); break;
             default: return set_error(QH_ERR_UNSUPPORTED, "decimation %d not supported", D);
             }
@@ -349,7 +375,10 @@
     else if (band2g) launch_band2g(a, ntiles, nl, stream, meter, egress);
     else if (a.mask_row && bnfft == kNfft) launch_band_rows<kNfft>(a, ntiles, nl, stream);
     else if (a.mask_row) launch_band_rows<kBandNfftMax>(a, ntiles, nl, stream);
-    else if (bnfft == kNfft) launch_band<kNfft>(a, ntiles, nl, stream, meter, egress);
+    else if (bnfft == kNfft && walk_now && QH_TILE_WALK_BAND && !list && !egress && a.tw_inv == a.tw_fwd) {
+        if (meter) launch_walk<1, true, false, false>(a, ntiles, nl, walk_grid(2), stream);
+        else launch_walk<1, false, false, false>(a, ntiles, nl, walk_grid(1), stream);
+    } else if (bnfft == kNfft) launch_band<kNfft>(a, ntiles, nl, stream, meter, egress);
     else launch_band<kBandNfftMax>(a, ntiles, nl, stream, meter, egress);
     tick(2);
     dim3 g((kHistBand + NT - 1) / NT, (unsigned)(list ? nlist : nch));
@@ -563,6 +592,7 @@
 
 int Engine::run_linear(ChainCall &k)
 {
+    struct WalkScope { bool &f; WalkScope(bool &f_, bool on) : f(f_) { f = on; } ~WalkScope() { f = false; } } walk_scope(walk_now, tile_walk);
     const long long n_mid = k.n_mid;
     const int nstage = 1 + (k.any_nbp ? 1 : 0) + (k.any_eqp ? 1 : 0) + (k.any_bp1 ? 1 : 0);
     int stage = 0, which = 0;
diff --git a/quisk_amd/csrc/qh_engine.hpp b/quisk_amd/csrc/qh_engine.hpp
--- a/quisk_amd/csrc/qh_engine.hpp
+++ b/quisk_amd/csrc/qh_engine.hpp
@@ -171,6 +171,10 @@
     bool band6k = false;
     int dbg_forms = [] { const char *e = std::getenv("QH_DBG_FORMS"); return e ? std::atoi(e) : 0; }();
     int band_tile_pref = 0;
+    bool tile_walk = true, walk_now = false;
+    int tile_walk_cap = 0;
+    int walk_res[3] = { 0, 0, 0 };
+    int walk_grid(int i) const { return tile_walk_cap > 0 && tile_walk_cap < walk_res[i] ? tile_walk_cap : walk_res[i]; }
     std::vector<cd> band_mask(const std::vector<cd> &h) const;
     unsigned long long *nco_phase = nullptr, *nco_dphase = nullptr, *nco_parked = nullptr;
     double2 *nco_step = nullptr;
diff --git a/quisk_amd/csrc/qh_engine_params.hip b/quisk_amd/csrc/qh_engine_params.hip
--- a/quisk_amd/csrc/qh_engine_params.hip
+++ b/quisk_amd/csrc/qh_engine_params.hip
@@ -1751,13 +1751,13 @@
     }
     std::vector<ChanCfg> keep_cfg;
     for (const ChanCfg &c : cfg) keep_cfg.push_back(settings_of(c, new_dsp));
-    static_assert(sizeof(Engine) == 9336, "Engine changed: see to Engine::rebuild's Wide and carried state, then update the size");
+    static_assert(sizeof(Engine) == 9360, "Engine changed: see to Engine::rebuild's Wide and carried state, then update the size");
     struct Wide {
         int device, nch; hipStream_t stream; bool own_stream; unsigned long long epoch;
-        bool graph_on; long long graph_launches; bool timing, meters_on; int band_tile_pref, snba_ovrlp; std::vector<SnbaTune> snba_tune_h;
+        bool graph_on; long long graph_launches; bool timing, meters_on; int band_tile_pref, snba_ovrlp; bool tile_walk; int tile_walk_cap; std::vector<SnbaTune> snba_tune_h;
         qh_ana *disp; int disp_ss, pll_check_only, agc_form;
         bool emnr_tables; std::vector<double> h_GG, h_GGS, h_zeta; std::vector<int> h_zeta_true; double h_zrange[4];
-    } was{ device, nch, stream, own_stream, epoch, graph_on, graph_launches, timing, meters_on, band_tile_pref, snba_ovrlp, snba_tune_h,
+    } was{ device, nch, stream, own_stream, epoch, graph_on, graph_launches, timing, meters_on, band_tile_pref, snba_ovrlp, tile_walk, tile_walk_cap, snba_tune_h,
            disp, disp_ss, pll_check_only, agc_form, emnr_tables, std::move(h_GG), std::move(h_GGS), std::move(h_zeta), std::move(h_zeta_true),
            { h_zrange[0], h_zrange[1], h_zrange[2], h_zrange[3] } };
     own_stream = false;
@@ -1767,7 +1767,7 @@
     in_rate = new_in; dsp_rate = new_dsp; out_rate = new_out; dsp_size = new_size; D = new_D;
     int rc = init();
     graph_on = was.graph_on; graph_launches = was.graph_launches; timing = was.timing; meters_on = was.meters_on;
-    band_tile_pref = was.band_tile_pref; snba_ovrlp = was.snba_ovrlp; snba_tune_h = was.snba_tune_h; snba_tune_dirty = true;
+    band_tile_pref = was.band_tile_pref; snba_ovrlp = was.snba_ovrlp; tile_walk = was.tile_walk; tile_walk_cap = was.tile_walk_cap; snba_tune_h = was.snba_tune_h; snba_tune_dirty = true;
     disp = was.disp; disp_ss = was.disp_ss; pll_check_only = was.pll_check_only; agc_form = was.agc_form;
     emnr_tables = was.emnr_tables; h_GG = std::move(was.h_GG); h_GGS = std::move(was.h_GGS); h_zeta = std::move(was.h_zeta); h_zeta_true = std::move(was.h_zeta_true);
     std::copy(was.h_zrange, was.h_zrange + 4, h_zrange);
diff --git a/quisk_amd/csrc/qh_fft.hpp b/quisk_amd/csrc/qh_fft.hpp
--- a/quisk_amd/csrc/qh_fft.hpp
+++ b/quisk_amd/csrc/qh_fft.hpp
@@ -151,10 +151,10 @@
 }
 
 template <int N, int R, bool INV, typename C>
-__device__ __forceinline__ void pass_regs_to_lds(C (&x)[R], C *lds)
+__device__ __forceinline__ void pass_regs_to_lds(C (&x)[R], C *lds, int tid = threadIdx.x)
 {
     static_assert(R == N / NT, "first pass radix must equal N/NT");
-    const int j = threadIdx.x;
+    const int j = tid;
     Dft<R, INV, C>::run(x);
     if constexpr (16 % R == 0) {
         C *p = lds + lds_phys(j * R);
@@ -174,7 +174,7 @@
 };
 
 template <int N, int R, int Ns, bool INV, typename C>
-__device__ __forceinline__ void pass_lds_to_lds(C *lds, const C (&w1)[PassGeom<N, R>::PER])
+__device__ __forceinline__ void pass_lds_to_lds(C *lds, const C (&w1)[PassGeom<N, R>::PER], int tid = threadIdx.x)
 {
     constexpr int NB = PassGeom<N, R>::NB;
     constexpr int PER = PassGeom<N, R>::PER;
@@ -183,7 +183,7 @@
     static_assert(NB % 16 == 0, "pass geometry");
 #pragma unroll
     for (int p = 0; p < PER; p++) {
-        int j = threadIdx.x + p * NT;
+        int j = tid + p * NT;
         if (NB >= NT || j < NB) {
             const C *q = lds + lds_phys(j);
 #pragma unroll
@@ -192,13 +192,13 @@
     }
 #pragma unroll
     for (int p = 0; p < PER; p++) {
-        int j = threadIdx.x + p * NT;
+        int j = tid + p * NT;
         if (NB >= NT || j < NB) base[p] = stockham_butterfly<N, R, Ns, INV>(x[p], j, w1[p]);
     }
     __syncthreads();
 #pragma unroll
     for (int p = 0; p < PER; p++) {
-        int j = threadIdx.x + p * NT;
+        int j = tid + p * NT;
         if (NB >= NT || j < NB) {
             if constexpr (Ns % 16 == 0) {
                 C *q = lds + lds_phys(base[p]);
@@ -217,10 +217,10 @@
 }
 
 template <int N, int R, bool INV, typename C>
-__device__ __forceinline__ void pass_lds_to_regs(const C *lds, C (&x)[R], C w1)
+__device__ __forceinline__ void pass_lds_to_regs(const C *lds, C (&x)[R], C w1, int tid = threadIdx.x)
 {
     static_assert(R == N / NT, "last pass radix must equal N/NT");
-    const int j = threadIdx.x;
+    const int j = tid;
     const C *q = lds + lds_phys(j);
 #pragma unroll
     for (int r = 0; r < R; r++) x[r] = q[r * (NT + NT / 16)];
@@ -316,11 +316,12 @@
     }
 
     template <int D>
-    static __device__ __forceinline__ void run_poly(C (&x)[16], void *lds_raw, const Tw &t)
+    static __device__ __forceinline__ void run_poly(C (&x)[16], void *lds_raw, const Tw &t) { run_poly_at<D>(x, lds_raw, t, threadIdx.x); }
+    template <int D>
+    static __device__ __forceinline__ void run_poly_at(C (&x)[16], void *lds_raw, const Tw &t, int j)
     {
         static_assert(!INV && (D == 2 || D == 4 || D == 8), "forward transform of a decimating stage");
         constexpr int R3 = 16 / D;
-        const int j = threadIdx.x;
         T *lds = reinterpret_cast<T *>(lds_raw);
         Dft<16, INV, C>::run(x);
         if constexpr (kSwizzle) exchange_sw<1>(x, lds, j, 0);
@@ -512,6 +513,34 @@
         static_assert(kSplit, "polyphase plan: the fp64 4096-point transform");
         FftSplit4096<INV, C>::template run_poly<D>(x, lds, t);
     }
+    static __device__ __forceinline__ void run_at(C (&x)[N / NT], void *lds, const Tw &t, int tid)
+    {
+        if constexpr (kSplit) {
+            FftSplit4096<INV, C>::run_at(x, lds, t, tid);
+        } else {
+            static_assert(N == 1024, "lane index handed over: the 1024-point plan only");
+            FftRR<N, INV, C>::first(x, reinterpret_cast<C *>(lds), tid);
+            FftRR<N, INV, C>::rest(reinterpret_cast<C *>(lds), x, t, tid);
+        }
+    }
+    template <int D> static __device__ __forceinline__ void run_poly_at(C (&x)[N / NT], void *lds, const Tw &t, int tid)
+    {
+        static_assert(kSplit, "polyphase plan: the fp64 4096-point transform");
+        FftSplit4096<INV, C>::template run_poly_at<D>(x, lds, t, tid);
+    }
+    static __device__ __forceinline__ Tw load_at(const C *__restrict__ tw, int tid)
+    {
+        if constexpr (N == 4096) return FftRR<N, INV, C>::load_at(tw, tid);
+        else {
+            static_assert(N == 1024, "lane index handed over: the 1024-point plan only");
+            Tw t;
+            t.a[0] = pass_twiddle<4, INV>(tw, tid);
+            t.b[0] = pass_twiddle<16, INV>(tw + 4, tid);
+            t.c[0] = pass_twiddle<64, INV>(tw + 20, tid);
+            t.d = pass_twiddle<256, INV>(tw + 84, tid);
+            return t;
+        }
+    }
 };
 
 template <bool INV, typename C> struct FftRR<2048, INV, C> {
@@ -548,17 +577,17 @@
         t.d = pass_twiddle<256, INV>(tw + 84, threadIdx.x);
         return t;
     }
-    static __device__ __forceinline__ void first(C (&x)[4], C *lds) { pass_regs_to_lds<1024, 4, INV>(x, lds); }
-    static __device__ __forceinline__ void rest(C *lds, C (&x)[4], const Tw &t)
-    {
-        __syncthreads();
-        pass_lds_to_lds<1024, 4, 4, INV>(lds, t.a);
-        __syncthreads();
-        pass_lds_to_lds<1024, 4, 16, INV>(lds, t.b);
-        __syncthreads();
-        pass_lds_to_lds<1024, 4, 64, INV>(lds, t.c);
-        __syncthreads();
-        pass_lds_to_regs<1024, 4, INV>(lds, x, t.d);
+    static __device__ __forceinline__ void first(C (&x)[4], C *lds, int tid = threadIdx.x) { pass_regs_to_lds<1024, 4, INV>(x, lds, tid); }
+    static __device__ __forceinline__ void rest(C *lds, C (&x)[4], const Tw &t, int tid = threadIdx.x)
+    {
+        __syncthreads();
+        pass_lds_to_lds<1024, 4, 4, INV>(lds, t.a, tid);
+        __syncthreads();
+        pass_lds_to_lds<1024, 4, 16, INV>(lds, t.b, tid);
+        __syncthreads();
+        pass_lds_to_lds<1024, 4, 64, INV>(lds, t.c, tid);
+        __syncthreads();
+        pass_lds_to_regs<1024, 4, INV>(lds, x, t.d, tid);
     }
 };
 
diff --git a/quisk_amd/csrc/qh_osfir.hpp b/quisk_amd/csrc/qh_osfir.hpp
--- a/quisk_amd/csrc/qh_osfir.hpp
+++ b/quisk_amd/csrc/qh_osfir.hpp
@@ -116,9 +116,8 @@
 #ifndef QH_XCD_SWIZZLE
 #define QH_XCD_SWIZZLE 1
 #endif
-__device__ __forceinline__ void xcd_tile_map(int ntiles, int &chan_slot, int &tile)
-{
-    const unsigned G = gridDim.x, lin = blockIdx.x;
+__device__ __forceinline__ void xcd_tile_entry(unsigned lin, unsigned G, int ntiles, int &chan_slot, int &tile)
+{
 #if QH_XCD_SWIZZLE
     const unsigned c = lin & 7u, k = lin >> 3, q = G >> 3, rem = G & 7u;
     const unsigned gt = c * q + (c < rem ? c : rem) + k;
@@ -128,6 +127,10 @@
 #endif
     chan_slot = (int)(gt / (unsigned)ntiles);
     tile = (int)(gt - (unsigned)chan_slot * (unsigned)ntiles);
+}
+__device__ __forceinline__ void xcd_tile_map(int ntiles, int &chan_slot, int &tile)
+{
+    xcd_tile_entry(blockIdx.x, gridDim.x, ntiles, chan_slot, tile);
 }
 
 template <typename T, int NFFT, int D, bool METER = false> constexpr int osfir_lds_bytes()
@@ -554,6 +557,168 @@
     }
 }
 
+#ifndef QH_TILE_WALK_FRONT
+#define QH_TILE_WALK_FRONT 1
+#endif
+#ifndef QH_TILE_WALK_BAND
+#define QH_TILE_WALK_BAND 0
+#endif
+#ifndef QH_WALK_CARRY_FRONT
+#define QH_WALK_CARRY_FRONT 2
+#endif
+#ifndef QH_WALK_CARRY_BAND
+#define QH_WALK_CARRY_BAND 0
+#endif
+template <typename T, int NFFT, int D, bool METER, bool OUTMIX, bool POLY>
+__global__ __launch_bounds__(NT, 4) void osfir_walk_kernel(OsfirArgs<T> a, int total)
+{
+    using C = cplx<T>;
+    constexpr int E = NFFT / NT, NOUT = NFFT / D, EO = E / D;
+    static_assert(E % D == 0 && EO >= 1 && NOUT >= 2 * NT && E <= 32, "see osfir_kernel");
+    static_assert(!METER || D == 1, "meters ride on a plain D = 1 stage");
+    static_assert(!METER || NT / 64 * kMeterLdsDoublesPerWave * 8 <= osfir_lds_bytes<T, NFFT, D, true>(), "meter blocks overlay the exchange image");
+    using Fwd = TileFft<NFFT, false, C>;
+    using Inv = TileFft<NOUT, true, C>;
+    extern __shared__ __align__(16) unsigned char smem[];
+    void *lds = smem;
+
+    const int t = threadIdx.x;
+    constexpr int kCarry = D == 1 ? QH_WALK_CARRY_BAND : QH_WALK_CARRY_FRONT;
+    using InvRaw = TileFft<NOUT, false, C>;
+    typename Fwd::Tw twf;
+    typename Inv::Tw twi;
+    typename InvRaw::Tw twr;
+    static_assert(sizeof(twr) == sizeof(twi), "one layout");
+    double mw = 0.0;
+    if constexpr (kCarry & 1) twf = Fwd::load(a.tw_fwd);
+    if constexpr ((kCarry & 2) && D > 1) twr = InvRaw::load_at(a.tw_inv, t);
+    if constexpr ((kCarry & 4) && METER) mw = a.meter_w[t & 63];
+    auto keep = [](auto &tw) {
+        double *d = reinterpret_cast<double *>(&tw);
+#pragma unroll
+        for (int i = 0; i < (int)(sizeof(tw) / sizeof(double)); i++) asm volatile("" : "+v"(d[i]));
+    };
+    auto again = [](auto *p) { asm volatile("" : "+s"(p)); return p; };
+    const int j0 = a.P / D;
+#ifdef QH_WALK_STAGGER
+    for (unsigned q = (blockIdx.x * 4u / gridDim.x) & 3u; q; q--) __builtin_amdgcn_s_sleep(95);
+#endif
+
+#pragma unroll 1
+    for (unsigned lin = blockIdx.x; lin < (unsigned)total; lin += gridDim.x) {
+        int tile, slot;
+        xcd_tile_entry(lin, (unsigned)total, a.ntiles, slot, tile);
+        const int ch = a.chan_list ? a.chan_list[slot] : slot;
+        const C *in = a.in + (long long)ch * a.in_stride;
+        const C *hist = a.hist ? a.hist + (long long)ch * a.hist_stride : nullptr;
+        const int g0 = a.off - a.P + tile * (D * a.Lout);
+        int tl = t;
+        asm volatile("" : "+v"(tl));
+
+        C x[E];
+        if ((g0 >= 0) && (g0 + NFFT <= a.n_in)) {
+            const C *p = in + g0 + tl;
+#pragma unroll
+            for (int r = 0; r < E; r++) x[r] = p[r * NT];
+        } else {
+            const unsigned ok = load_tile<T, E>(x, in, hist, a.hist_len, a.n_in, g0);
+#pragma unroll
+            for (int r = 0; r < E; r++)
+                if (!((ok >> r) & 1u)) x[r] = mk<T>(0, 0);
+        }
+        if constexpr (METER) {
+            if constexpr (kCarry & 4) keep(mw); else mw = again(a.meter_w)[tl & 63];
+            meter_tap<C, E>(x, a.P >> 8, mw, reinterpret_cast<double *>(lds) + (tl >> 6) * kMeterLdsDoublesPerWave, a.meter_in + (long long)ch * a.meter_stride + (long long)tile * (a.Lout >> 6), tl >> 6, tl & 63);
+            __syncthreads();
+        }
+
+        if constexpr (kCarry & 1) keep(twf); else twf = Fwd::load_at(again(a.tw_fwd), tl);
+        if constexpr (POLY) Fwd::template run_poly_at<D>(x, lds, twf, tl);
+        else Fwd::run_at(x, lds, twf, tl);
+
+        const C *mask = a.mask + (long long)ch * a.mask_stride;
+        C z[EO];
+#pragma unroll
+        for (int i = 0; i < EO; i++) {
+            C acc = cmul(x[i], mask[tl + NT * i]);
+#pragma unroll
+            for (int q = 1; q < D; q++) acc = cadd(acc, cmul(x[i + EO * q], mask[tl + NT * (i + EO * q)]));
+            z[i] = acc;
+            if (((i + 1) * D) % QH_MASK_BATCH == 0) __builtin_amdgcn_sched_barrier(0);
+        }
+
+        __syncthreads();
+        int te = t;
+        asm volatile("" : "+v"(te));
+        if constexpr ((kCarry & 1) && D == 1) { twi.a[0] = cconj(twf.a[0]); twi.b = cconj(twf.b); }
+        else if constexpr ((kCarry & 2) && D > 1) {
+            keep(twr);
+            const C *raw = reinterpret_cast<const C *>(&twr);
+            C *cj = reinterpret_cast<C *>(&twi);
+#pragma unroll
+            for (int i = 0; i < (int)(sizeof(twi) / sizeof(C)); i++) cj[i] = cconj(raw[i]);
+        }
+        else twi = Inv::load_at(again(a.tw_inv), te);
+        Inv::run_at(z, lds, twi, te);
+        if constexpr (METER) {
+            __syncthreads();
+            if constexpr (kCarry & 4) keep(mw); else mw = again(a.meter_w)[te & 63];
+            meter_tap<C, EO>(z, a.P >> 8, mw, reinterpret_cast<double *>(lds) + (te >> 6) * kMeterLdsDoublesPerWave, a.meter_out + (long long)ch * a.meter_stride + (long long)tile * (a.Lout >> 6), te >> 6, te & 63);
+        }
+
+        if constexpr (OUTMIX) {
+            const double2 tr = a.tile_rot[(long long)ch * a.ntiles + tile];
+            const double2 st = a.nco_step[ch];
+            const double2 lr = a.lane_rot[(long long)ch * NT + te];
+            const C step = mk<T>((T)st.x, (T)st.y);
+            C rot = cmul(mk<T>((T)tr.x, (T)tr.y), mk<T>((T)lr.x, (T)lr.y));
+#pragma unroll
+            for (int i = 0; i < EO; i++) {
+                z[i] = cmul(z[i], rot);
+                if (i + 1 < EO) rot = cmul(rot, step);
+            }
+        }
+
+        C *out = a.out + (long long)ch * a.out_stride + a.out_offset;
+        EpiParam ep;
+        if (a.epi) ep = a.epi[ch]; else { ep.a = 1; ep.b = 0; ep.c = 0; ep.d = 1; }
+        if (a.pick <= 1) {
+#pragma unroll
+            for (int i = 0; i < EO; i++) {
+                const int rel = te + NT * i - j0;
+                const long long m = (long long)tile * a.Lout + rel;
+                if (rel >= 0 && rel < a.Lout && m < a.n_out) {
+                    C v;
+                    v.x = (T)ep.a * z[i].x + (T)ep.b * z[i].y;
+                    v.y = (T)ep.c * z[i].x + (T)ep.d * z[i].y;
+                    out[m] = v;
+                }
+            }
+        } else {
+            const int lpt = a.Lout / a.pick;
+#pragma unroll
+            for (int i = 0; i < EO; i++) {
+                const int rel = te + NT * i - j0;
+                const int q = rel / a.pick;
+                const long long m = (long long)tile * lpt + q;
+                if (rel >= 0 && rel < a.Lout && q * a.pick == rel && m < a.n_out) {
+                    C v;
+                    v.x = (T)ep.a * z[i].x + (T)ep.b * z[i].y;
+                    v.y = (T)ep.c * z[i].x + (T)ep.d * z[i].y;
+                    out[m] = v;
+                }
+            }
+        }
+        if (a.hist_next && g0 + NFFT > a.n_in - a.hist_len) {
+            C *hn = a.hist_next + (long long)ch * a.hist_stride;
+            const int first = a.n_in - a.hist_len;
+#pragma unroll 1
+            for (int g = max(g0, first) + te; g < min(g0 + NFFT, a.n_in); g += NT) hn[g - first] = in[g];
+        }
+        if constexpr (!METER) lds_barrier();
+    }
+}
+
 __device__ __forceinline__ double2 sel2(bool c, double2 a, double2 b) { return make_double2(c ? a.x : b.x, c ? a.y : b.y); }
 constexpr int kOsfir8kThreads = 512, kOsfir8kP = 2048, kOsfir8kLout = 6144;
 constexpr int kOsfir8kImage = FftSplit4096<false, double2>::kLdsBytes > 4 * 2 * 64 * 9 * 8 ? FftSplit4096<false, double2>::kLdsBytes : 4 * 2 * 64 * 9 * 8;
diff --git a/quisk_amd/csrc/qh_rxa_api.hip b/quisk_amd/csrc/qh_rxa_api.hip
--- a/quisk_amd/csrc/qh_rxa_api.hip
+++ b/quisk_amd/csrc/qh_rxa_api.hip
@@ -773,6 +773,16 @@
 }
 int qh_rxa_band_tile(const qh_rxa *h) { return h ? h->e.bnfft : 0; }
 
+int qh_rxa_set_tile_walk(qh_rxa *h, int on, int max_workgroups)
+{
+    if (!h || (on != 0 && on != 1) || max_workgroups < 0) return set_error(QH_ERR_INVALID, "qh_rxa_set_tile_walk: on = 0 or 1, max_workgroups >= 0 (0: all that are resident)");
+    QH_RXA_LOCK(h);
+    h->e.tile_walk = on != 0;
+    h->e.tile_walk_cap = max_workgroups;
+    h->e.epoch++;
+    return QH_OK;
+}
+
 int qh_rxa_process_packed(qh_rxa *h, const void *d_src, long long src_bytes, const qh_iq_format *fmt, long long chan_stride,
                           double *d_out, long long out_stride, int nblk)
 {
diff --git a/quisk_amd/lib.py b/quisk_amd/lib.py
--- a/quisk_amd/lib.py
+++ b/quisk_amd/lib.py
@@ -107,6 +107,7 @@
     L.qh_rxa_set_graph_replay.argtypes = [vp, i]
     L.qh_rxa_set_band_tile.argtypes = [vp, i]
     L.qh_rxa_band_tile.argtypes = [vp]
+    L.qh_rxa_set_tile_walk.argtypes = [vp, i, i]
     L.qh_rxa_graph_launches.argtypes = [vp]
     L.qh_rxa_graph_launches.restype = ll
     L.qh_rxa_pll_repairs.argtypes = [vp]
diff --git a/quisk_amd/rxa.py b/quisk_amd/rxa.py
--- a/quisk_amd/rxa.py
+++ b/quisk_amd/rxa.py
@@ -236,6 +236,9 @@
     def band_tile(self):
         return self._L.qh_rxa_band_tile(self._h)
 
+    def set_tile_walk(self, on=True, max_workgroups=0):
+        check(self._L.qh_rxa_set_tile_walk(self._h, 1 if on else 0, int(max_workgroups)))
+
     def graph_launches(self):
         return self._L.qh_rxa_graph_launches(self._h)
 
```

New measurement: 129,400 Mcomplex-samples/s. -11.8%, worse.
